# MadNLP/MadNLP.jl

Measured on AMD Instinct MI355X. Metric: IP iterations/sec + ms per factorize!/solve!, condensed KKT n≈1e4, higher is better.
Workload: dtype f64; 1 GPU; BASELINE config C3: case1354pegase-shaped sparse-condensed KKT, one instance; N=11192, m=16646, nnz(K)=68688; step = compress_J+compress_H+build_kkt+factorize (n_f=1) + inertia fetch + 2 solve_linear_system per instance; algorithm=BUNCHKAUFMAN (device: static-pivot LDL^T), outer_block=0, batch_per_gpu=1, batch_api=n/a (one instance), parallelism=1 GPU(s) x 1 independent instance(s)

## Files before the change

include/madnlp_hip.h:

```cpp
#ifndef MADNLP_HIP_H
#define MADNLP_HIP_H

#include <stdint.h>

#ifdef __cplusplus
extern "C" {
#endif

#define MNK_VERSION 100

enum { MNK_HOST = 0, MNK_DEVICE = 1 };

enum { MNK_BUNCHKAUFMAN = 1, MNK_LU = 2, MNK_QR = 3, MNK_CHOLESKY = 4, MNK_LDL = 5, MNK_EVD = 6 };

typedef struct mnk_ctx mnk_ctx;
typedef struct mnk_sc mnk_sc;
typedef struct mnk_dc mnk_dc;
typedef struct mnk_ls mnk_ls;

int mnk_version(void);
const char* mnk_last_error_string(void);
int mnk_ctx_create(int device, void* stream, mnk_ctx** out);
int mnk_ctx_destroy(mnk_ctx* ctx);
int mnk_ctx_synchronize(mnk_ctx* ctx);
// ... 193 lines not shown
int mnk_ipm_vec_copy(mnk_ipm* ipm, double* dst, const double* src, int64_t n);
int mnk_ipm_vec_fill(mnk_ipm* ipm, double* v, int64_t n, double value);
int mnk_ipm_vec_axpby(mnk_ipm* ipm, double* out, double a, const double* x, double b, const double* y, int64_t n);
int mnk_ipm_vec_scatter_axpy(mnk_ipm* ipm, double* y, const int64_t* idx, double a, const double* x, int64_t n);
int mnk_ipm_vec_gather(mnk_ipm* ipm, double* out, double a, const double* x, const int64_t* idx, int64_t n);
int mnk_ipm_bound_dual_axpy(mnk_ipm* ipm, double* zl, double* zu, double a, const double* dzl, const double* dzu);
int mnk_ipm_bound_dual_fill(mnk_ipm* ipm, double* zl, double* zu, double v);
int mnk_ipm_gemv(mnk_ipm* ipm, int trans, int64_t m, int64_t n, double alpha, const double* A, int64_t lda, const double* x,
                 double beta, double* y);

int mnk_ipm_vec_mul(mnk_ipm* ipm, double* out, const double* a, const double* b, int64_t n);
int mnk_ipm_scale_cons(mnk_ipm* ipm, double* c, const double* con_scale, const double* slack, const int64_t* slack_pos,
                       int64_t ns, const double* rhs, int64_t m);
int mnk_ipm_scale_grad(mnk_ipm* ipm, double* f, int64_t n, int64_t ntot, double factor);

typedef struct mnk_opf mnk_opf;
int mnk_opf_create(mnk_ctx* ctx, int64_t nbus, int64_t ngen, int64_t nbranch, const int32_t* fr, const int32_t* to,
                   const int32_t* gen_bus, const double* arc_coef, const double* bus_data, const double* gen_cost,
                   mnk_opf** out);
int mnk_opf_destroy(mnk_opf* opf);
int mnk_opf_sizes(mnk_opf* opf, int64_t* n, int64_t* m, int64_t* nnzj, int64_t* nnzh);
int mnk_opf_obj_terms(mnk_opf* opf, const double* x, double* terms );
int mnk_opf_grad(mnk_opf* opf, const double* x, double* g);
int mnk_opf_cons(mnk_opf* opf, const double* x, double* c);
int mnk_opf_jac_coord(mnk_opf* opf, const double* x, double* jac);
int mnk_opf_hess_coord(mnk_opf* opf, const double* x, const double* y, double obj_weight, double* hess);

typedef struct mnk_tape mnk_tape;
int mnk_tape_create(mnk_ctx* ctx, int64_t n, int64_t m, void* out);
int mnk_tape_destroy(void* tape);
int mnk_tape_add_pattern(void* tape, int kind , int64_t R, int k, int q,
                         const int32_t* var_index, const double* params, const int32_t* rows,
                         int64_t ninstr0, const int32_t* code0, int64_t nconst0, const double* consts0, int64_t nout0,
                         const int32_t* out_operand0, const int32_t* out_j0, const int32_t* out_l0, int nslot0,
                         int64_t ninstr1, const int32_t* code1, int64_t nconst1, const double* consts1, int64_t nout1,
                         const int32_t* out_operand1, const int32_t* out_j1, const int32_t* out_l1, int nslot1,
                         int64_t ninstr2, const int32_t* code2, int64_t nconst2, const double* consts2, int64_t nout2,
                         const int32_t* out_operand2, const int32_t* out_j2, const int32_t* out_l2, int nslot2);
int mnk_tape_finalize(void* tape);
int mnk_tape_sizes(void* tape, int64_t* n, int64_t* m, int64_t* nterms, int64_t* nnzj, int64_t* nnzh);
int mnk_tape_extended(void* tape, int* mask);
int mnk_tape_get_structure(void* tape, int32_t* jac_I, int32_t* jac_J, int32_t* hess_I, int32_t* hess_J);
int mnk_tape_obj_terms(void* tape, const double* x, double* terms );
int mnk_tape_grad(void* tape, const double* x, double* g);
int mnk_tape_cons(void* tape, const double* x, double* c);
int mnk_tape_jac_coord(void* tape, const double* x, double* jac);
int mnk_tape_hess_coord(void* tape, const double* x, const double* y, double obj_weight, double* hess);

typedef struct mnk_schur mnk_schur;
int mnk_schur_create(mnk_ctx* ctx, int64_t ns_local, int64_t blk, int64_t nd, int algo, mnk_schur** out);
int mnk_schur_destroy(mnk_schur* h);
int mnk_schur_set_block(mnk_schur* h, int64_t k, const double* A_kk, int64_t lda, const double* C_dk, int64_t ldc,
                        int loc);
int mnk_schur_build_local(mnk_schur* h, const double* S0, int64_t lds0, int loc_s0, double* S_out, int64_t lds_out);
int mnk_schur_factorize_s(mnk_schur* h, const double* S, int64_t lds, int loc, int* info);
int mnk_schur_inertia_s(mnk_schur* h, int64_t* num_pos, int64_t* num_zero, int64_t* num_neg);
int mnk_schur_scenario_inertia(mnk_schur* h, int64_t k, int64_t* num_pos, int64_t* num_zero, int64_t* num_neg);
int mnk_schur_scenario_bk_info(mnk_schur* h, int64_t k, int* active, int* count);
int mnk_schur_forward(mnk_schur* h, double* rhs_k, double* contrib_d);
int mnk_schur_solve_s(mnk_schur* h, double* rhs_d);
int mnk_schur_backward(mnk_schur* h, double* rhs_k, const double* x_d);
void* mnk_schur_s_buffer(mnk_schur* h);
int mnk_schur_set_structure(mnk_schur* h, int64_t n, int64_t m, int64_t nv, int64_t nc, int64_t nnzh, const int32_t* hess_I,
                            const int32_t* hess_J, int64_t nnzj, const int32_t* jac_I, const int32_t* jac_J, int64_t n_ineq,
                            const int64_t* ind_ineq, int64_t n_eq, const int64_t* ind_eq, int index_base, int64_t ns_global,
                            const int64_t* local_scen, int own_design);
int mnk_schur_assemble(mnk_schur* h, const double* hess, const double* jac, const double* pr_diag, const double* du_diag, int loc);
void* mnk_schur_s0_buffer(mnk_schur* h);
int mnk_schur_get_block(mnk_schur* h, int64_t k, double* A_kk, double* C_dk, double* S0);
int mnk_schur_solve(mnk_schur* h, double* rhs_k, double* rhs_d, int loc);

int mnk_ls_debug_solve_trace(mnk_ls* ls, unsigned long long* out, int64_t n);

int mnk_ls_debug_dag_state(mnk_ls* ls, int* flags, int64_t nflags, int* chain, int64_t nchain, int* have);

int mnk_debug_grid_at_launch(int cu_first, int num_cu, int first, int per_cu);
int mnk_debug_shader_clock(mnk_ctx* ctx, double* mhz);

int mnk_debug_dag_tasks(int ntile, int chunk, int band_tiles, int js2, int taper0, int* out, int cap, int* first_phase);
int mnk_debug_dag_merged_tasks(int ntile, int chunk, int band_tiles, int js2, int taper0, int fill, int ninst, int period,
                               int* out, int cap);
int mnk_debug_dag_deal(int ntile, int chunk, int band_tiles, int js2, int taper0, int fill, int ninst, int period, int nq, int gang,
                       int* tasks_out, int* order, int cap, int* off, int* first_phase);

int mnk_sc_debug_tile_env(mnk_sc* sc, int64_t order, int32_t* out, int cap);
int mnk_debug_tile_env_csc(int64_t n, const int32_t* colptr, const int32_t* rowval, int index_base, int32_t* out, int cap);
int mnk_sc_debug_tile_envh(mnk_sc* sc, int64_t order, int32_t* out, int cap);
int mnk_debug_tile_envh_csc(int64_t n, const int32_t* colptr, const int32_t* rowval, int index_base, int32_t* out, int cap);
int mnk_debug_envh_ksteps(int ntile, int chunk, int band_tiles, int js2, int taper0, const int* env, const int* envh, int64_t* count);

#ifdef __cplusplus
}
#endif
#endif
```

madnlp.jl_amd/_lib.py:

```python
from __future__ import annotations

import ctypes as C
import os
import subprocess

_HERE = os.path.dirname(os.path.abspath(__file__))
CSRC = os.path.join(_HERE, "csrc")
LIBDIR = os.path.join(_HERE, "lib")
LIBPATH = os.path.join(LIBDIR, "libmadnlp_hip.so")
_LIB_OVERRIDE = os.environ.get("MNK_LIBPATH")
SOURCES = ["gemm_f64.hip", "dag.hip", "factor.hip", "solve.hip", "ls.hip", "sparse_kkt.hip", "dense_kkt.hip", "bk.hip", "schur.hip", "ipm_vec.hip", "opf_eval.hip", "qr.hip", "lu.hip", "evd.hip", "qn.hip", "tape_eval.hip", "nlp_scale.hip"]
HEADERS = ["common.h", "ls.h", "kkt_vec.h", "gemm_tile.h", "leaf64.h", "ipm_handle.h", os.path.join("..", "..", "include", "madnlp_hip.h")]

MNK_HOST, MNK_DEVICE = 0, 1
MNK_BUNCHKAUFMAN, MNK_LU, MNK_QR, MNK_CHOLESKY, MNK_LDL, MNK_EVD = 1, 2, 3, 4, 5, 6
MNK_SC_JT, MNK_SC_HESS, MNK_SC_AUG, MNK_SC_DIAGBUF = 0, 1, 2, 3
MNK_QN_BFGS, MNK_QN_DAMPED_BFGS = 1, 2


def _stale() -> bool:
    if not os.path.exists(LIBPATH):
        return True
    t = os.path.getmtime(LIBPATH)
    deps = [os.path.join(CSRC, s) for s in SOURCES + HEADERS]
# ... 128 lines not shown
    "mnk_ipm_populate_RR_nn": (C.c_int, [_vp, _vp, _vp, C.c_int64, C.c_double, C.c_double]),
    "mnk_ipm_initialize_robust_restorer": (C.c_int, [_vp, _vp, _vp, C.c_int64, C.c_double, C.c_double, _vp, _vp, _vp, _vp, _vp, _vp, _vp, _vp]),
    "mnk_ipm_set_f_RR": (C.c_int, [_vp, _vp, _vp, _vp, _vp, C.c_double]),
    "mnk_ipm_set_aug_rhs_RR": (C.c_int, [_vp, _vp, _vp, _vp, _vp, _vp, _vp, _vp, _vp, _vp, _vp, C.c_int64, _vp, _vp, _vp, C.c_double, C.c_double, _vp, _vp, _vp, _vp]),
    "mnk_ipm_finish_aug_solve_RR": (C.c_int, [_vp, _vp, _vp, _vp, _vp, _vp, _vp, _vp, _vp, _vp, _vp, C.c_int64, C.c_double, C.c_double]),
    "mnk_ipm_reset_bound_dual_1": (C.c_int, [_vp, _vp, _vp, C.c_int64, C.c_double, C.c_double]),
    "mnk_ipm_set_initial_bounds": (C.c_int, [_vp, _vp, _vp, C.c_int64, C.c_double]),
    "mnk_ipm_set_initial_rhs": (C.c_int, [_vp, _vp, _vp, _vp, _vp, _vp, C.c_int64, _vp, _vp]),
    "mnk_ipm_set_aug_rhs_ifr": (C.c_int, [_vp, _vp, C.c_int64, _vp, _vp, _vp, _vp]),
    "mnk_ipm_set_g_ifr": (C.c_int, [_vp, _vp, _vp, _vp, _vp, _vp, _vp, C.c_double]),
    "mnk_ipm_initialize_variables": (C.c_int, [_vp, _vp, _vp, _vp, C.c_int64, C.c_double, C.c_double]),
    "mnk_ipm_get_dot": (C.c_int, [_vp, _vp, _vp, C.c_int64, C.POINTER(C.c_double)]),
    "mnk_ipm_get_sum": (C.c_int, [_vp, _vp, C.c_int64, C.POINTER(C.c_double)]),
    "mnk_ipm_get_norm2": (C.c_int, [_vp, _vp, C.c_int64, C.POINTER(C.c_double)]),
    "mnk_ipm_vec_copy": (C.c_int, [_vp, _vp, _vp, C.c_int64]),
    "mnk_ipm_vec_fill": (C.c_int, [_vp, _vp, C.c_int64, C.c_double]),
    "mnk_ipm_vec_axpby": (C.c_int, [_vp, _vp, C.c_double, _vp, C.c_double, _vp, C.c_int64]),
    "mnk_ipm_vec_scatter_axpy": (C.c_int, [_vp, _vp, _vp, C.c_double, _vp, C.c_int64]),
    "mnk_ipm_vec_gather": (C.c_int, [_vp, _vp, C.c_double, _vp, _vp, C.c_int64]),
    "mnk_ipm_bound_dual_axpy": (C.c_int, [_vp, _vp, _vp, C.c_double, _vp, _vp]),
    "mnk_ipm_bound_dual_fill": (C.c_int, [_vp, _vp, _vp, C.c_double]),
    "mnk_ipm_gemv": (C.c_int, [_vp, C.c_int, C.c_int64, C.c_int64, C.c_double, _vp, C.c_int64, _vp, C.c_double, _vp]),
    "mnk_ipm_vec_mul": (C.c_int, [_vp, _vp, _vp, _vp, C.c_int64]),
    "mnk_ipm_scale_cons": (C.c_int, [_vp, _vp, _vp, _vp, _vp, C.c_int64, _vp, C.c_int64]),
    "mnk_ipm_scale_grad": (C.c_int, [_vp, _vp, C.c_int64, C.c_int64, C.c_double]),
    "mnk_opf_create": (C.c_int, [_vp, C.c_int64, C.c_int64, C.c_int64, _vp, _vp, _vp, _vp, _vp, _vp, C.POINTER(_vp)]),
    "mnk_opf_destroy": (C.c_int, [_vp]),
    "mnk_opf_sizes": (C.c_int, [_vp, _i64p, _i64p, _i64p, _i64p]),
    "mnk_opf_obj_terms": (C.c_int, [_vp, _vp, _vp]),
    "mnk_opf_grad": (C.c_int, [_vp, _vp, _vp]),
    "mnk_opf_cons": (C.c_int, [_vp, _vp, _vp]),
    "mnk_opf_jac_coord": (C.c_int, [_vp, _vp, _vp]),
    "mnk_opf_hess_coord": (C.c_int, [_vp, _vp, _vp, C.c_double, _vp]),
    "mnk_tape_create": (C.c_int, [_vp, C.c_int64, C.c_int64, _vp]),
    "mnk_tape_destroy": (C.c_int, [_vp]),
    "mnk_tape_add_pattern": (C.c_int, [_vp, C.c_int, C.c_int64, C.c_int, C.c_int, _vp, _vp, _vp]
                             + [C.c_int64, _vp, C.c_int64, _vp, C.c_int64, _vp, _vp, _vp, C.c_int] * 3),
    "mnk_tape_finalize": (C.c_int, [_vp]),
    "mnk_tape_sizes": (C.c_int, [_vp, _i64p, _i64p, _i64p, _i64p, _i64p]),
    "mnk_tape_extended": (C.c_int, [_vp, _vp]),
    "mnk_tape_get_structure": (C.c_int, [_vp, _vp, _vp, _vp, _vp]),
    "mnk_tape_obj_terms": (C.c_int, [_vp, _vp, _vp]),
    "mnk_tape_grad": (C.c_int, [_vp, _vp, _vp]),
    "mnk_tape_cons": (C.c_int, [_vp, _vp, _vp]),
    "mnk_tape_jac_coord": (C.c_int, [_vp, _vp, _vp]),
    "mnk_tape_hess_coord": (C.c_int, [_vp, _vp, _vp, C.c_double, _vp]),
    "mnk_sc_set_aug_RR": (C.c_int, [_vp, _vp, _vp, _vp, _vp, _vp, _vp, _vp, _vp, _vp, _vp, C.c_double, C.c_double, C.c_double]),
    "mnk_dc_set_aug_RR": (C.c_int, [_vp, _vp, _vp, _vp, _vp, _vp, _vp, _vp, _vp, _vp, _vp, C.c_double, C.c_double, C.c_double]),
    "mnk_ls_bk_info": (C.c_int, [_vp, C.POINTER(C.c_int), C.POINTER(C.c_int), _vp, _vp]),
    "mnk_ls_get_stat": (C.c_int, [_vp, C.c_char_p, C.POINTER(C.c_double)]),
    "mnk_sc_set_bounds": (C.c_int, [_vp, C.c_int64, _vp, C.c_int64, _vp, C.c_int]),
    "mnk_sc_set_barrier_terms": (C.c_int, [_vp, _vp, _vp, _vp, _vp, _vp, C.c_int]),
    "mnk_sc_solve_kkt": (C.c_int, [_vp, _vp, _vp, C.c_int]),
    "mnk_sc_mul": (C.c_int, [_vp, _vp, _vp, C.c_double, C.c_double, C.c_int]),
    "mnk_dc_set_bounds": (C.c_int, [_vp, C.c_int64, _vp, C.c_int64, _vp, C.c_int]),
    "mnk_dc_set_barrier_terms": (C.c_int, [_vp, _vp, _vp, _vp, _vp, _vp, C.c_int]),
    "mnk_dc_solve_kkt": (C.c_int, [_vp, _vp, _vp, C.c_int]),
    "mnk_dc_mul": (C.c_int, [_vp, _vp, _vp, C.c_double, C.c_double, C.c_int]),
    "mnk_schur_create": (C.c_int, [_vp, C.c_int64, C.c_int64, C.c_int64, C.c_int, C.POINTER(_vp)]),
    "mnk_schur_destroy": (C.c_int, [_vp]),
    "mnk_schur_set_block": (C.c_int, [_vp, C.c_int64, _vp, C.c_int64, _vp, C.c_int64, C.c_int]),
    "mnk_schur_build_local": (C.c_int, [_vp, _vp, C.c_int64, C.c_int, _vp, C.c_int64]),
    "mnk_schur_factorize_s": (C.c_int, [_vp, _vp, C.c_int64, C.c_int, C.POINTER(C.c_int)]),
    "mnk_schur_inertia_s": (C.c_int, [_vp, _i64p, _i64p, _i64p]),
    "mnk_schur_scenario_inertia": (C.c_int, [_vp, C.c_int64, _i64p, _i64p, _i64p]),
    "mnk_schur_scenario_bk_info": (C.c_int, [_vp, C.c_int64, C.POINTER(C.c_int), C.POINTER(C.c_int)]),
    "mnk_schur_forward": (C.c_int, [_vp, _vp, _vp]),
    "mnk_schur_solve_s": (C.c_int, [_vp, _vp]),
    "mnk_schur_backward": (C.c_int, [_vp, _vp, _vp]),
    "mnk_schur_s_buffer": (C.c_void_p, [_vp]),
    "mnk_schur_set_structure": (C.c_int, [_vp, C.c_int64, C.c_int64, C.c_int64, C.c_int64, C.c_int64, _vp, _vp, C.c_int64, _vp, _vp,
                                          C.c_int64, _vp, C.c_int64, _vp, C.c_int, C.c_int64, _vp, C.c_int]),
    "mnk_schur_assemble": (C.c_int, [_vp, _vp, _vp, _vp, _vp, C.c_int]),
    "mnk_schur_s0_buffer": (_vp, [_vp]),
    "mnk_schur_get_block": (C.c_int, [_vp, C.c_int64, _vp, _vp, _vp]),
    "mnk_schur_solve": (C.c_int, [_vp, _vp, _vp, C.c_int]),
    "mnk_ls_debug_solve_trace": (C.c_int, [_vp, _vp, C.c_int64]),
    "mnk_ls_debug_dag_state": (C.c_int, [_vp, _vp, C.c_int64, _vp, C.c_int64, _vp]),
    "mnk_debug_grid_at_launch": (C.c_int, [C.c_int, C.c_int, C.c_int, C.c_int]),
    "mnk_debug_shader_clock": (C.c_int, [_vp, _vp]),
    "mnk_debug_dag_tasks": (C.c_int, [C.c_int, C.c_int, C.c_int, C.c_int, C.c_int, _vp, C.c_int, _vp]),
    "mnk_debug_dag_merged_tasks": (C.c_int, [C.c_int] * 8 + [_vp, C.c_int]),
    "mnk_debug_dag_deal": (C.c_int, [C.c_int] * 10 + [_vp, _vp, C.c_int, _vp, _vp]),
    "mnk_sc_debug_tile_env": (C.c_int, [_vp, C.c_int64, _vp, C.c_int]),
    "mnk_debug_tile_env_csc": (C.c_int, [C.c_int64, _vp, _vp, C.c_int, _vp, C.c_int]),
    "mnk_sc_debug_tile_envh": (C.c_int, [_vp, C.c_int64, _vp, C.c_int]),
    "mnk_debug_tile_envh_csc": (C.c_int, [C.c_int64, _vp, _vp, C.c_int, _vp, C.c_int]),
    "mnk_debug_envh_ksteps": (C.c_int, [C.c_int] * 5 + [_vp, _vp, _vp]),
    "mnk_factorize_batch_begin": (C.c_int, []),
    "mnk_factorize_batch_end": (C.c_int, []),
    "mnk_solve_batch_begin": (C.c_int, []),
    "mnk_solve_batch_end": (C.c_int, []),
    "mnk_release_idle_streams": (C.c_int, [C.c_int]),
    "mnk_sc_step_batch": (C.c_int, [C.c_int, _vp, _vp, _vp, _vp, _vp, _vp, C.c_int]),
    "mnk_ls_inertia_batch": (C.c_int, [C.c_int, _vp, _i64p, _i64p, _i64p]),
    "mnk_ls_solve_batch": (C.c_int, [C.c_int, _vp, _vp, C.c_int]),
    "mnk_gemm_nt": (C.c_int, [_vp, C.c_int, C.c_int64, C.c_int64, C.c_int64, _vp, C.c_int64, _vp,
                              C.c_int64, _vp, C.c_int64]),
}


def lib():
    global _lib
    if _lib is not None:
        return _lib
    if not os.path.exists(LIBPATH):
        raise ImportError(
            f"{LIBPATH} is missing: run `python -c 'import __graft_entry__ as g; g.build()'` "
            "(hipcc --offload-arch=gfx950).  There is no CPU fallback for the KKT hot path.")
    try:
        import torch
    except Exception:
        pass
    l = C.CDLL(_LIB_OVERRIDE if _LIB_OVERRIDE and os.path.exists(_LIB_OVERRIDE) else LIBPATH)
    for name, (res, args) in SIGNATURES.items():
        f = getattr(l, name)
        f.restype = res
        f.argtypes = args
    _lib = l
    return l


class HipError(RuntimeError):
    pass


def check(rc: int, what: str = ""):
    if rc != 0:
        msg = lib().mnk_last_error_string()
        raise HipError(f"{what} failed (rc={rc}): {msg.decode() if msg else ''}")
```

madnlp.jl_amd/csrc/common.h:

```cpp
#pragma once
#include <hip/hip_runtime.h>
#include <cstdint>
#include <cstdlib>
#include <cstdio>
#include <cstring>
#include <mutex>
#include <string>
#include <vector>

#include "../../include/madnlp_hip.h"

namespace mnk {

void set_error(const char* fmt, ...);

#define MNK_HIP(call)                                                                   \
    do {                                                                                \
        hipError_t e_ = (call);                                                         \
        if (e_ != hipSuccess) {                                                         \
            mnk::set_error("%s:%d: %s -> %s", __FILE__, __LINE__, #call, hipGetErrorString(e_)); \
            return -2;                                                                  \
        }                                                                               \
    } while (0)

// ... 91 lines not shown
    void release() {
        if (p) {
            LaunchLock lock;
            quiesce_persistent();
            (void)hipFree(p);
        }
        p = nullptr;
        n = 0;
    }
    ~DevBuf() { release(); }
};

}

struct mnk_ctx {
    int device = 0;
    hipStream_t stream = nullptr;
    bool own_stream = false;
    hipStream_t sp = nullptr, su = nullptr;
    int panel_cus = 0;
    hipStream_t sp_dag = nullptr, su_dag = nullptr;
    hipStream_t sp_dagB = nullptr, su_dagB = nullptr;
    bool shared_dag_streams = false;
    int dag_cus = 0;
    hipStream_t sp_dag2 = nullptr, su_dag2 = nullptr;
    int dag_cus2 = 0;
    hipEvent_t ev_a = nullptr, ev_b = nullptr;
    hipStream_t s_fill = nullptr;
    std::vector<hipEvent_t> ev_panel, ev_next, ev_next2, ev_bdone;
    int num_cu = 256;
    int cu_first = 0;
    int total_cu = 256;
    bool partitioned = false;
    void* persist_slot = nullptr;
    int children = 0;
    bool released = false;
};
int mnk_masked_stream_pair(mnk_ctx* ctx, int chain_cus, hipStream_t* sp, hipStream_t* su);
int mnk_ctx_ensure_panel_streams(mnk_ctx* ctx);
int mnk_ctx_ensure_dag(mnk_ctx* ctx);
int mnk_ctx_ensure_dag2(mnk_ctx* ctx);
int mnk_ctx_ensure_batch_streams(mnk_ctx* ctx);
int mnk_solve_warmup(hipStream_t s);
int mnk_ctx_bulk_wgs(const mnk_ctx* ctx, int first, int per_cu);
int mnk_dag_warmup(hipStream_t* streams, int n, int nwg);
int mnk_live_contexts(int device);
int mnk_persist_begin(mnk_ctx* ctx, hipStream_t s);
int mnk_persist_end(mnk_ctx* ctx, hipStream_t s, int rc);
void mnk_ctx_child_added(mnk_ctx* ctx);
void mnk_ctx_child_gone(mnk_ctx* ctx);

namespace mnk {
struct PpDag {
    int* front;
    const int* af;
    int ntile;
    int need_front;
    int front_from;
    int af_tilecol;
    long spin_limit;
    unsigned long long* trace;
    unsigned long long* vmax;
    int* dbg;
};
}

namespace mnk {

int launch_gemm_nt(hipStream_t s, int mode, int64_t M, int64_t N, int64_t K,
                   const double* A, int64_t lda, const double* B, int64_t ldb,
                   double* C, int64_t ldc, const double* colscale, double* C2, int64_t ldc2,
                   const int* info_flag);
struct TrsmBatchRec { double* X; double* V; const double* dblk; const double* inv16; const double* dinv; const int* info; };
struct GemmBatchRec { const double* A; const double* B; double* C; const int* info; };
int launch_gemm_nt_batch(hipStream_t s, int64_t M, int64_t N, int64_t K, const GemmBatchRec* recs_dev, int nbatch, int64_t lda,
                         int64_t ldb, int64_t ldc);
int launch_gemm_nt_lower_small(hipStream_t s, int64_t M, int64_t N, int64_t K, const double* A, int64_t lda,
                               const double* B, int64_t ldb, double* C, int64_t ldc, const int* info_flag);
int gemm_nt_lower_tiles(int64_t M, int64_t N);
int launch_gemm_nt_queue(hipStream_t s, int64_t M, int64_t N, int64_t K, const double* A, int64_t lda,
                         const double* B, int64_t ldb, double* C, int64_t ldc, int* counter, int cus,
                         const int* info_flag);

int dag_build_tasks(int ntile, int chunk, int band_tiles, int js2, std::vector<int>& out, int taper0, std::vector<int>* ready);
int dag_add_fill_tasks(int ntile, std::vector<int>& tasks, std::vector<int>& ready, int n1);
void dag_merge_tasks(const std::vector<int>& tasks, const std::vector<int>& ready, int ninst, int period, std::vector<int>& out);
constexpr int DAG_NQ = 8;
constexpr int DAG_QHEAD_STRIDE = 32;
constexpr int DAG_QHEAD_WORDS = (DAG_NQ + 1) * DAG_QHEAD_STRIDE;
void dag_deal_tasks(const std::vector<int>& tasks, const std::vector<int>& ready, int t0, int t1, int nq, int gang, std::vector<int>& order,
                    std::vector<int>& off);
void dag_envh_count(const std::vector<int>& tasks, const int* env, const int* envh, int nenv, int64_t* count);

}
```

madnlp.jl_amd/csrc/dag.hip:

```cpp
#include <algorithm>
#include <atomic>
#include <cfloat>
#include <climits>
#include <vector>

#include "gemm_tile.h"
#include "ls.h"

namespace mnk {


struct DagInst {
    double* F;
    int64_t ld;
    double* V;
    const double* dinv;
    const double* dblk;
    const double* inv16;
    int* front;
    int* af;
    int* tprog;
    int* info;
    unsigned long long* vmax;
    double* zfill;
// ... 356 lines not shown
            if (tr) { tr[4] = wall_clock64(); s_stat[1] += tr[4] - tr[3]; }
            dag_finalize_tile<LDL>(in, row0, col0, 2 * J, smem_raw, tid, X, tr);
            if (tr) s_stat[3] += wall_clock64() - tr[4];
        } else if (!(I == J && kend > k0)) {
            v4f64 acc[4][4];
#pragma unroll
            for (int i = 0; i < 4; ++i)
#pragma unroll
                for (int j = 0; j < 4; ++j) acc[i][j] = v4f64{0.0, 0.0, 0.0, 0.0};
            if (flags & DAG_FINAL) __builtin_amdgcn_s_setprio(3);
            if (!gemm_nt_mainloop<2, 2, 4, 8>(acc, Ak, in->ld, Bk, in->ld, (kend - k0) * 16, smem_raw, tid, gate)) return false;
            if (tr) tr[1] = wall_clock64();
            if (!wait_chunk_order()) return false;
            if (kend > k0)
                gemm_nt_epilogue<2, 2, 4, 2, false, true>(acc, row0, col0, (int64_t)1 << 40, (int64_t)1 << 40, in->F, in->ld, nullptr, nullptr, 0, tid);
            if (tr) tr[3] = wall_clock64();
        } else {
            v4f64 acc[4][4];
#pragma unroll
            for (int i = 0; i < 4; ++i)
#pragma unroll
                for (int j = 0; j < 4; ++j) acc[i][j] = v4f64{0.0, 0.0, 0.0, 0.0};
            __builtin_amdgcn_s_setprio(3);
            if (!wait_chunk_order()) return false;
            gemm_nt_load_neg_lower<2, 2, 4>(acc, row0, col0, in->F, in->ld, tid);
            if (!gemm_nt_mainloop<2, 2, 4, 8>(acc, Ak, in->ld, Bk, in->ld, (kend - k0) * 16, smem_raw, tid, gate)) return false;
            if (tr) tr[1] = wall_clock64();
            gemm_nt_store_neg_lower<2, 2, 4>(acc, row0, col0, in->F, in->ld, tid);
            if (tr) tr[3] = wall_clock64();
        }
        return true;
        };
        const bool done = run_task();
        asm volatile("s_waitcnt vmcnt(0)" ::: "memory");
        __syncthreads();
        if (done && tid == 0) {
            __builtin_amdgcn_fence(__ATOMIC_RELEASE, "agent");
            asm volatile("s_waitcnt vmcnt(0)" ::: "memory");
            if (!(flags & DAG_FINAL)) {
                __hip_atomic_store(in->tprog + (int64_t)I * a.ntile + J, q + 1, __ATOMIC_RELAXED, __HIP_MEMORY_SCOPE_AGENT);
            } else if (!(flags & DAG_BANDACC)) {
                __hip_atomic_store(in->front + 2 * I, J + 1, __ATOMIC_RELAXED, __HIP_MEMORY_SCOPE_AGENT);
                __hip_atomic_store(in->front + 2 * I + 1, J + 1, __ATOMIC_RELAXED, __HIP_MEMORY_SCOPE_AGENT);
            } else {
                __hip_atomic_store(in->af + (int64_t)I * a.ntile + J, 1, __ATOMIC_RELAXED, __HIP_MEMORY_SCOPE_AGENT);
            }
            if (tr) tr[5] = wall_clock64();
        }
        __builtin_amdgcn_s_setprio(0);
        __syncthreads();
        };
        do_task((DagInstP)(uintptr_t)(a.insts + inst));
    }
}

struct DagArgs1 {
    double* F;
    int64_t ld;
    double* V;
    const double* dinv;
    const double* dblk;
    const double* inv16;
    const int4* tasks;
    int ntasks;
    int* front;
    int* af;
    int* tprog;
    int ntile;
    int* qctr;
    int* info;
    long spin_limit;
    unsigned long long* trace;
    unsigned long long* wgstat;
    unsigned long long* vmax;
    int fake_share;
    double* zfill;
    int64_t N;
    const int* env;
    const int* envgate;
    const int* envh;
    const int* qoff;
    int* qheads;
    int nq;
};

__device__ __forceinline__ int dag_pop(const int* __restrict__ qoff, int* __restrict__ qheads, int nq, int* sq) {
    const int h = sq[0];
    if (h >= 0) {
        const int beg = qoff[h], n = qoff[h + 1] - beg;
        const int i = atomicAdd(qheads + h * DAG_QHEAD_STRIDE, 1);
        if (i < n) return beg + i;
        sq[0] = -1 - h;
    }
    for (;;) {
        int best = -1, most = 0;
        for (int x = 0; x < nq; ++x) {
            const int left = qoff[x + 1] - qoff[x] - __hip_atomic_load(qheads + x * DAG_QHEAD_STRIDE, __ATOMIC_RELAXED, __HIP_MEMORY_SCOPE_AGENT);
            if (left > most) { most = left; best = x; }
        }
        if (best < 0) return INT_MAX;
        const int i = atomicAdd(qheads + best * DAG_QHEAD_STRIDE, 1);
        if (i < qoff[best + 1] - qoff[best]) {
            sq[1] += 1;
            atomicAdd(qheads + nq * DAG_QHEAD_STRIDE, 1);
            return qoff[best] + i;
        }
    }
}

template <bool LDL>
__global__ __launch_bounds__(256, 3) void dag_bulk_kernel1(DagArgs1 a) {
    extern __shared__ __attribute__((aligned(16))) char smem_raw[];
    __shared__ int s_val;
    __shared__ int s_q[2];
    if (threadIdx.x == 0) {
        unsigned xcc;
        asm volatile("s_getreg_b32 %0, hwreg(HW_REG_XCC_ID)" : "=s"(xcc));
        s_q[0] = a.nq > 0 ? (int)(xcc & 15u) % a.nq : 0;
        s_q[1] = 0;
    }
    __shared__ unsigned long long s_stat[4];
    if (threadIdx.x < 4) s_stat[threadIdx.x] = 0;
    const int* __restrict__ env = a.env != nullptr && __builtin_amdgcn_readfirstlane(*a.envgate) == 0 ? a.env : nullptr;
    const int* __restrict__ envh = env != nullptr ? a.envh : nullptr;
    __syncthreads();
    for (;;) {
        int tid = threadIdx.x;
        asm volatile("" : "+v"(tid));
        if (tid == 0)
            s_val = __hip_atomic_load(a.info, __ATOMIC_RELAXED, __HIP_MEMORY_SCOPE_AGENT) != 0
                        ? INT_MAX
                        : (a.nq > 0 ? dag_pop(a.qoff, a.qheads, a.nq, s_q) : atomicAdd(a.qctr, 1));
        __syncthreads();
        const int t = s_val;
        __syncthreads();
        if (t >= a.ntasks) {
            if (a.wgstat != nullptr && tid == 0) {
                unsigned long long* w = a.wgstat + (int64_t)blockIdx.x * 8;
                w[0] = s_stat[0]; w[1] = wall_clock64(); w[2] = s_stat[1]; w[3] = s_stat[2]; w[4] = s_stat[3];
                w[5] = a.nq > 0 ? (unsigned long long)(1 + (s_q[0] >= 0 ? s_q[0] : -1 - s_q[0])) : 0; w[6] = (unsigned long long)s_q[1];
            }
            return;
        }
        if (a.wgstat != nullptr && tid == 0) { if (s_stat[0] == 0) s_stat[0] = wall_clock64(); ++s_stat[2]; }
        const int4 tk = a.tasks[t];
        const int flags = __builtin_amdgcn_readfirstlane(tk.x) & 255, q = __builtin_amdgcn_readfirstlane(tk.x) >> 8;
        const int I = __builtin_amdgcn_readfirstlane(tk.y), J = __builtin_amdgcn_readfirstlane(tk.z) & 0xfff;
        const int kbeg = __builtin_amdgcn_readfirstlane(tk.w) & 0xffff, kend = __builtin_amdgcn_readfirstlane(tk.w) >> 16;
        const int64_t row0 = (int64_t)128 * I, col0 = (int64_t)128 * J;
        unsigned long long* tr = a.trace != nullptr && tid == 0
                                     ? a.trace + (int64_t)(a.nq > 0 ? (int)((unsigned)__builtin_amdgcn_readfirstlane(tk.z) >> 12) : t) * 8
                                     : nullptr;
        if (tr) { tr[0] = wall_clock64(); tr[6] = 0; tr[7] = 0; }
        if (flags & DAG_FILL) {
            if (a.zfill != nullptr) dag_fill_tile(&a, I, J, tid);
            continue;
        }

        int eI = 0, k0 = kbeg;
        if (env != nullptr) {
            eI = __builtin_amdgcn_readfirstlane(env[I]);
            k0 = min(kend, max(kbeg, max(eI, __builtin_amdgcn_readfirstlane(env[J]))));
        }
        int kf = 0, ks = 0;
        if (envh != nullptr && (!(flags & DAG_FINAL) || (flags & DAG_BANDACC))) {
            const int w = __builtin_amdgcn_readfirstlane(tid >> 6);
            const int hI0 = __builtin_amdgcn_readfirstlane(envh[2 * I]), hI1 = __builtin_amdgcn_readfirstlane(envh[2 * I + 1]);
            const int hJ0 = __builtin_amdgcn_readfirstlane(envh[2 * J]), hJ1 = __builtin_amdgcn_readfirstlane(envh[2 * J + 1]);
            ks = min(max(8 * max(min(hI0, hI1), min(hJ0, hJ1)) - 16 * k0, 0), 16 * (kend - k0));
            kf = (I == J && w == 2) ? INT_MAX : 8 * max((w & 1) ? hI1 : hI0, (w >> 1) ? hJ1 : hJ0) - 16 * k0 - ks;
        }
        const int nk = 16 * (kend - k0) - ks;
        int limit = 0;
        auto gate_at = [&](int kc) -> int {
            const unsigned long long w0 = tr ? wall_clock64() : 0;
            const int r = dag_wait_front(&a, a.spin_limit, 2 * I, 2 * I + 1, 2 * J, 2 * J + 1, kc, kend, &s_val);
            if (tr) { const unsigned long long w1 = wall_clock64(); tr[2] = w1; tr[6] += 1; tr[7] += w1 - w0; s_stat[1] += w1 - w0; }
            return r;
        };
        auto gate = [&](int kt) -> bool {
            if (kt < limit) return true;
            const int r = gate_at(k0 + ((kt + ks) >> 4));
            if (r < 0) return false;
            limit = (__builtin_amdgcn_readfirstlane(r) - k0) * 16 - ks;
            return true;
        };
        const double* Ak = a.F + (a.fake_share > 0 ? (int64_t)128 * (kend + I % a.fake_share) : row0) + (int64_t)(128 * k0 + 8 * ks) * a.ld;
        const double* Bk = (LDL ? a.V : a.F) + (a.fake_share > 0 ? (int64_t)128 * (kend + J % a.fake_share) : col0) + (int64_t)(128 * k0 + 8 * ks) * a.ld;
        auto wait_chunk_order = [&]() -> bool {
            if (flags & DAG_FIRST) return true;
            const int* word = a.tprog + (int64_t)I * a.ntile + J;
            const unsigned long long w0 = tr ? wall_clock64() : 0;
            if (!dag_wait_words(&a, a.spin_limit, word, q, word, q, &s_val)) return false;
            if (tr) s_stat[1] += wall_clock64() - w0;
            return true;
        };
        if ((flags & DAG_FINAL) && !(flags & DAG_BANDACC)) {
            __builtin_amdgcn_s_setprio(3);
            if (!wait_chunk_order()) return;
            if (J < eI) {
                if (kend > kbeg && gate_at(kbeg) < 0) return;
                if (LDL) dag_zero_tile(a.V, a.ld, row0, col0, tid);
                goto publish;
            }
            v4f64 X[8][2];
            {
                const int lane = tid & 63, w = tid >> 6;
                const double* Cs = a.F + (row0 + 32 * w + (lane & 15)) + (col0 + (lane >> 4)) * a.ld;
#pragma unroll
                for (int cb = 0; cb < 8; ++cb)
#pragma unroll
                    for (int r = 0; r < 4; ++r) {
                        const double* cp = Cs + (int64_t)(16 * cb + 4 * r) * a.ld;
                        X[cb][0][r] = cp[0];
                        X[cb][1][r] = cp[16];
                    }
            }
            if (kend > kbeg && gate_at(kbeg) < 0) return;
            if (kend > k0) (void)gemm_nt_mainloop3<2, 8, true>(X, Ak, a.ld, Bk, a.ld, (kend - k0) * 16, smem_raw, tid);
#pragma unroll
            for (int i = 0; i < 8; ++i) { asm volatile("" : "+v"(X[i][0])); asm volatile("" : "+v"(X[i][1])); }
            if (tr) tr[1] = tr[3] = wall_clock64();
            if (dag_wait_front(&a, a.spin_limit, 2 * J, 2 * J + 1, 2 * J, 2 * J + 1, J, J + 1, &s_val) < 0) return;
            if (tr) { tr[4] = wall_clock64(); s_stat[1] += tr[4] - tr[3]; }
            dag_finalize_tile<LDL>(&a, row0, col0, 2 * J, smem_raw, tid, X, tr);
            if (tr) s_stat[3] += wall_clock64() - tr[4];
        } else if (!(I == J && kend > k0)) {
            v4f64 acc[4][4];
#pragma unroll
            for (int i = 0; i < 4; ++i)
#pragma unroll
                for (int j = 0; j < 4; ++j) acc[i][j] = v4f64{0.0, 0.0, 0.0, 0.0};
            if (flags & DAG_FINAL) __builtin_amdgcn_s_setprio(3);
            if (!gemm_nt_mainloop<2, 2, 4, 8>(acc, Ak, a.ld, Bk, a.ld, nk, smem_raw, tid, gate, kf)) return;
            if (tr) tr[1] = wall_clock64();
            if (!wait_chunk_order()) return;
            if (kend > k0 && kf < nk)
                gemm_nt_epilogue<2, 2, 4, 2, false, true>(acc, row0, col0, (int64_t)1 << 40, (int64_t)1 << 40, a.F, a.ld, nullptr, nullptr, 0, tid);
            if (tr) tr[3] = wall_clock64();
        } else {
            v4f64 acc[4][4];
#pragma unroll
            for (int i = 0; i < 4; ++i)
#pragma unroll
                for (int j = 0; j < 4; ++j) acc[i][j] = v4f64{0.0, 0.0, 0.0, 0.0};
            __builtin_amdgcn_s_setprio(3);
            if (!wait_chunk_order()) return;
            gemm_nt_load_neg_lower<2, 2, 4>(acc, row0, col0, a.F, a.ld, tid);
            if (!gemm_nt_mainloop<2, 2, 4, 8>(acc, Ak, a.ld, Bk, a.ld, nk, smem_raw, tid, gate, kf)) return;
            if (tr) tr[1] = wall_clock64();
            gemm_nt_store_neg_lower<2, 2, 4>(acc, row0, col0, a.F, a.ld, tid);
            if (tr) tr[3] = wall_clock64();
        }
    publish:
        asm volatile("s_waitcnt vmcnt(0)" ::: "memory");
        __syncthreads();
        if (tid == 0) {
            __builtin_amdgcn_fence(__ATOMIC_RELEASE, "agent");
            asm volatile("s_waitcnt vmcnt(0)" ::: "memory");
            if (!(flags & DAG_FINAL)) {
                __hip_atomic_store(a.tprog + (int64_t)I * a.ntile + J, q + 1, __ATOMIC_RELAXED, __HIP_MEMORY_SCOPE_AGENT);
            } else if (!(flags & DAG_BANDACC)) {
                __hip_atomic_store(a.front + 2 * I, J + 1, __ATOMIC_RELAXED, __HIP_MEMORY_SCOPE_AGENT);
                __hip_atomic_store(a.front + 2 * I + 1, J + 1, __ATOMIC_RELAXED, __HIP_MEMORY_SCOPE_AGENT);
            } else {
                __hip_atomic_store(a.af + (int64_t)I * a.ntile + J, 1, __ATOMIC_RELAXED, __HIP_MEMORY_SCOPE_AGENT);
            }
            if (tr) tr[5] = wall_clock64();
        }
        __builtin_amdgcn_s_setprio(0);
        __syncthreads();
    }
}

int dag_build_tasks(int ntile, int chunk, int band_tiles, int js2, std::vector<int>& out, int taper0, std::vector<int>* ready) {
    struct T { int ready, cls, J, I, flags, q, kbeg, kend; };
    std::vector<T> ts;
    auto add_tile = [&](int I, int J, int K, bool band) {
        const int body = band ? K : std::max(0, K - 1);
        std::vector<int> cuts{body};
        int e = body;
        for (int len = taper0; len < chunk && e > 0; len *= 2) { e = std::max(0, e - len); cuts.push_back(e); }
        const int first = 1 + (I * 5 + J * 3) % chunk;
        while (e > first) { e = std::max(first, e - chunk); cuts.push_back(e); }
        if (e > 0) cuts.push_back(0);
        int q = 0;
        for (int c = (int)cuts.size() - 1; c > 0; --c, ++q) {
            const int kb = cuts[c], ke = cuts[c - 1];
            const bool last = band && ke == K;
            ts.push_back({ke, band ? 0 : 2, J, I, (band ? DAG_BANDACC : 0) | (last ? DAG_FINAL : 0) | (q == 0 ? DAG_FIRST : 0), q, kb, ke});
        }
        if (!band) ts.push_back({K, 1, J, I, DAG_FINAL | (q == 0 ? DAG_FIRST : 0), q, body, K});
    };
    for (int Jt = 0; Jt < ntile; ++Jt) {
        const int Js = Jt / 2;
        const int bt = Js >= js2 ? ntile : band_tiles;
        for (int I = 2 * Js + bt; I < ntile; ++I) add_tile(I, Jt, Jt, false);
        if (2 * Js - 2 > 0)
            for (int I = std::max(2 * Js, Jt); I < 2 * Js + bt && I < ntile; ++I) add_tile(I, Jt, 2 * Js - 2, true);
    }
    std::stable_sort(ts.begin(), ts.end(), [](const T& x, const T& y) {
        if (x.ready != y.ready) return x.ready < y.ready;
        if (x.cls != y.cls) return x.cls < y.cls;
        if (x.J != y.J) return x.J < y.J;
        return x.I < y.I;
    });
    out.clear();
    out.reserve(ts.size() * 4);
    if (ready != nullptr) { ready->clear(); ready->reserve(ts.size()); }
    int n1 = 0;
    for (const T& t : ts) {
        if (t.ready <= 2 * js2) ++n1;
        if (ready != nullptr) ready->push_back(t.ready);
        out.push_back(t.flags | (t.q << 8));
        out.push_back(t.I);
        out.push_back(t.J);
        out.push_back(t.kbeg | (t.kend << 16));
    }
    return n1;
}

int dag_add_fill_tasks(int ntile, std::vector<int>& tasks, std::vector<int>& ready, int n1) {
    const int nt = (int)(tasks.size() / 4), nfill = ntile * (ntile + 1) / 2;
    const int span = n1 > 0 ? n1 : nt;
    if (span <= 0) return n1;
    std::vector<int> out, rdy;
    out.reserve(tasks.size() + 4 * (size_t)nfill);
    rdy.reserve(ready.size() + nfill);
    int fi = 0, fj = 0, done = 0;
    auto emit_fill = [&](int r) {
        out.push_back(DAG_FILL); out.push_back(fi); out.push_back(fj); out.push_back(0);
        rdy.push_back(r);
        if (++fi >= ntile) { ++fj; fi = fj; }
        ++done;
    };
    for (int t = 0; t < nt; ++t) {
        for (int k = 0; k < 4; ++k) out.push_back(tasks[4 * t + k]);
        rdy.push_back(ready[t]);
        if (t < span)
            while (done < (int)((int64_t)(t + 1) * nfill / span)) emit_fill(ready[t]);
    }
    tasks.swap(out);
    ready.swap(rdy);
    return n1 > 0 ? n1 + nfill : 0;
}

void dag_merge_tasks(const std::vector<int>& tasks, const std::vector<int>& ready, int ninst, int period, std::vector<int>& out) {
    const int nt = (int)ready.size();
    out.clear();
    out.reserve((size_t)ninst * nt * 4);
    std::vector<int> pos(ninst, 0);
    for (;;) {
        int best = -1;
        long bkey = 0;
        for (int i = 0; i < ninst; ++i) {
            if (pos[i] >= nt) continue;
            const long key = (long)i * period + ready[pos[i]];
            if (best < 0 || key < bkey) { best = i; bkey = key; }
        }
        if (best < 0) break;
        const int t = pos[best]++;
        out.push_back(tasks[4 * t]);
        out.push_back(tasks[4 * t + 1] | (best << 16));
        out.push_back(tasks[4 * t + 2]);
        out.push_back(tasks[4 * t + 3]);
    }
}

void dag_deal_tasks(const std::vector<int>& tasks, const std::vector<int>& ready, int t0, int t1, int nq, int gang, std::vector<int>& order,
                    std::vector<int>& off) {
    nq = std::max(nq, 1);
    std::vector<std::vector<int>> qs(nq);
    std::vector<int64_t> load(nq, 0);
// ... 2 lines not shown
    auto ksteps = [&](int t) { return (tasks[4 * (size_t)t] & DAG_FILL) ? 0 : (tasks[4 * (size_t)t + 3] >> 16) - (tasks[4 * (size_t)t + 3] & 0xffff); };
    auto same = [&](int x, int y) {
        return ready[x] == ready[y] && cls(x) == cls(y) && tasks[4 * (size_t)x + 2] == tasks[4 * (size_t)y + 2] &&
               tasks[4 * (size_t)x + 3] == tasks[4 * (size_t)y + 3] && (tasks[4 * (size_t)x + 1] >> 16) == (tasks[4 * (size_t)y + 1] >> 16);
    };
    auto deal = [&](int b, int e) {
        int q = 0;
        if (gang >= 0) {
            q = rr % nq;
            for (int i = 1; i < nq; ++i)
                if (load[(rr + i) % nq] < load[q]) q = (rr + i) % nq;
            rr = q + 1;
        }
        for (int t = b; t < e; ++t) { qs[q].push_back(t); load[q] += ksteps(t); }
    };
    for (int i = t0; i < t1;) {
        int j = i + 1;
        const int c = cls(i);
        if (gang > 1 && (c == 0 || c == 2))
            while (j < t1 && same(i, j)) ++j;
        for (int b = i; b < j; b += std::max(gang, 1)) deal(b, std::min(j, b + std::max(gang, 1)));
        i = j;
    }
    order.clear();
    off.assign(1, 0);
    for (int q = 0; q < nq; ++q) {
        order.insert(order.end(), qs[q].begin(), qs[q].end());
        off.push_back((int)order.size());
    }
}

void dag_envh_count(const std::vector<int>& tasks, const int* env, const int* envh, int nenv, int64_t* count) {
    count[0] = count[1] = 0;
    for (size_t t = 0; t + 3 < tasks.size(); t += 4) {
        const int flags = tasks[t] & 255, I = tasks[t + 1] & 0xffff, J = tasks[t + 2] & 0xfff, kb = tasks[t + 3] & 0xffff, ke = tasks[t + 3] >> 16;
        if (flags & DAG_FILL) continue;
        const bool in = env != nullptr && I < nenv && J < nenv;
        const int k0 = in ? std::min(ke, std::max(kb, std::max(env[I], env[J]))) : kb;
        if (in && (flags & DAG_FINAL) && !(flags & DAG_BANDACC) && J < env[I]) continue;
        count[0] += 8 * (int64_t)(ke - k0);
        if (!in || envh == nullptr || ((flags & DAG_FINAL) && !(flags & DAG_BANDACC))) continue;
        for (int r = 0; r < 2; ++r)
            for (int c = 0; c < 2; ++c) {
                const int h0 = (I == J && r == 0 && c == 1) ? 2 * ke : std::max(envh[2 * I + r], envh[2 * J + c]);
                count[1] += std::min(2 * ke, std::max(2 * k0, h0)) - 2 * k0;
            }
    }
}

template <bool LDL>
static int launch_bulk_t(hipStream_t s, const DagArgs& a, int nwg) {
    const size_t smem = TILE3_LDS_BYTES;
    auto kern = dag_bulk_kernel<LDL>;
    static std::atomic<uint64_t> attr_devs{0};
    int dev = 0;
    MNK_HIP(hipGetDevice(&dev));
    if (!(attr_devs.load(std::memory_order_relaxed) >> (dev & 63) & 1)) {
        MNK_HIP(hipFuncSetAttribute((const void*)kern, hipFuncAttributeMaxDynamicSharedMemorySize, (int)smem));
        attr_devs.fetch_or(1ull << (dev & 63), std::memory_order_relaxed);
    }
    hipLaunchKernelGGL(kern, dim3(nwg), dim3(256), smem, s, a);
    MNK_HIP(hipGetLastError());
    return 0;
}

template <bool LDL>
static int launch_bulk1_t(hipStream_t s, const DagArgs1& a, int nwg) {
    const size_t smem = TILE3_LDS_BYTES;
    auto kern = dag_bulk_kernel1<LDL>;
    static std::atomic<uint64_t> attr_devs{0};
    int dev = 0;
    MNK_HIP(hipGetDevice(&dev));
    if (!(attr_devs.load(std::memory_order_relaxed) >> (dev & 63) & 1)) {
        MNK_HIP(hipFuncSetAttribute((const void*)kern, hipFuncAttributeMaxDynamicSharedMemorySize, (int)smem));
        attr_devs.fetch_or(1ull << (dev & 63), std::memory_order_relaxed);
    }
    hipLaunchKernelGGL(kern, dim3(nwg), dim3(256), smem, s, a);
    MNK_HIP(hipGetLastError());
    return 0;
}

static int launch_dag_bulk(hipStream_t s, bool ldl, const DagInst& one, const DagInst* insts, const int* tasks, int ntasks, int ntile,
                           int* qctr, long spin_limit, int nwg, unsigned long long* trace, unsigned long long* wgstat,
                           const int* qoff = nullptr, int* qheads = nullptr, int nq = 0) {
    if (ntasks <= 0) return 0;
    static const int fake = getenv("MNK_DAG_FAKE_SHARE") ? atoi(getenv("MNK_DAG_FAKE_SHARE")) : 0;
    if (insts == nullptr) {
        DagArgs1 a{one.F, one.ld, one.V, one.dinv, one.dblk, one.inv16, reinterpret_cast<const int4*>(tasks), ntasks, one.front, one.af,
                   one.tprog, ntile, qctr, one.info, spin_limit, trace, wgstat, one.vmax, fake, one.zfill, one.N, one.env, one.envgate, one.envh,
                   qoff, qheads, nq};
        return ldl ? launch_bulk1_t<true>(s, a, nwg) : launch_bulk1_t<false>(s, a, nwg);
    }
    DagArgs a{insts, reinterpret_cast<const int4*>(tasks), ntasks, ntile, qctr, spin_limit, trace, wgstat, fake};
    return ldl ? launch_bulk_t<true>(s, a, nwg) : launch_bulk_t<false>(s, a, nwg);
}

}

using namespace mnk;

int mnk_dag_warmup(hipStream_t* streams, int n, int nwg) {
    static mnk::DevBuf<int> ctr;
    if (!ctr.p) {
        if (ctr.alloc(4)) return -2;
        MNK_HIP(hipMemset(ctr.p, 0, 4 * sizeof(int)));
    }
    for (int i = 0; i < n; ++i) {
        if (streams[i] == nullptr) continue;
        mnk::DagArgs1 a1{};
        a1.qctr = ctr.p;
        a1.info = ctr.p + 1;
        mnk::DagArgs a{};
        a.qctr = ctr.p;
        int rc = mnk::launch_bulk1_t<true>(streams[i], a1, nwg);
        if (!rc) rc = mnk::launch_bulk1_t<false>(streams[i], a1, nwg);
        if (!rc) rc = mnk::launch_bulk_t<true>(streams[i], a, nwg);
        if (!rc) rc = mnk::launch_bulk_t<false>(streams[i], a, nwg);
        if (rc) return rc;
    }
    for (int i = 0; i < n; ++i)
        if (streams[i] != nullptr) MNK_HIP(mnk::stream_wait(streams[i]));
    return 0;
}

long mnk_ls_dag_spin_limit(const mnk_ls* ls) {
    if (ls->dag_spin_limit > 0) return ls->dag_spin_limit;
    const double n = (double)ls->Np;
    const double t_est = n * n * n / 3.0 / 50e12;
    const double polls = 10.0 * t_est / 0.17e-6;
    const double floor_polls = mnk_live_contexts(ls->ctx->device) > 1 ? 5880000.0 : 588000.0;
    return (long)std::min(16777216.0, std::max(floor_polls, polls));
}

static int bulk_xcds(const mnk_ctx* c, int first) {
    bool has[8] = {false, false, false, false, false, false, false, false};
    for (int b = std::max(first, 0); b < c->num_cu; ++b) has[(c->cu_first + b) % 8] = true;
    int n = 0;
    for (bool x : has) n += x ? 1 : 0;
    return n;
}

static mnk::DagInst dag_instance(mnk_ls* ls) {
    const int ntile = (int)(ls->Np / 128), nblk = (int)(ls->Np / NBI);
    int* front = ls->dag_flags.p + 2;
    int* af = front + nblk;
    int* tprog = af + (size_t)ntile * ntile;
    double* zfill = (ls->dag_fill && ls->dag_has_fill && ls->spare_pending && ls->fact_spare.p && !ls->spare_zeroed) ? ls->fact_spare.p : nullptr;
    const bool env = ls->envelope && ls->env_dev != nullptr && ls->env_word.p != nullptr;
    return mnk::DagInst{ls->fact.p, ls->ld, ls->algo == MNK_LDL ? ls->vfull.p : nullptr, ls->dinv.p, ls->dblk.p, ls->inv16.p,
                        front, af, tprog, ls->info_dev.p, mnk_ls_growth_word(ls), zfill, ls->N, env ? ls->env_dev : nullptr,
                        env ? ls->env_word.p + 1 : nullptr, env && ls->envelope_half ? ls->envh_dev : nullptr};
}

int mnk_ls_dag_prepare(mnk_ls* ls) {
    mnk_ctx* ctx = ls->ctx;
    hipStream_t s = ctx->stream;
    const int64_t Np = ls->Np, ld = ls->ld;
    const bool ldl = ls->algo == MNK_LDL;
    const int ntile = (int)(Np / 128), nblk = (int)(Np / NBI), nsc = (int)((Np + 255) / 256);
    const size_t nflags = (size_t)2 + nblk + 2 * (size_t)ntile * ntile;
    auto give_up = [&]() {
        (void)hipGetLastError();
        ls->dag_tasks.release();
        ls->dag_flags.release();
        ls->dag_qoff.release();
        ls->dag_qheads.release();
        ls->vfull.release();
        return 1;
    };
    if (!ls->dag_tasks.p) {
        const int64_t deep_rows = std::min<int64_t>((int64_t)ctx->dag_cus2 * NBI, ls->dag_deep_rows);
        ls->dag_js2 = (ctx->dag_cus2 > 0 && Np <= deep_rows) ? 0 : nsc;
        if (ls->dag_js2_override >= 0) ls->dag_js2 = std::min(nsc, ls->dag_js2_override);
        std::vector<int>& h = ls->dag_host_tasks;
        ls->dag_ntasks1 = mnk::dag_build_tasks(ntile, ls->dag_chunk, ls->dag_band / 2, ls->dag_js2, h, ls->dag_taper0, &ls->dag_host_ready);
        ls->dag_has_fill = ls->dag_fill && ls->prefill && Np <= mnk_ls::PREFILL_MAX_ROWS;
        if (ls->dag_has_fill && h.empty()) ls->dag_has_fill = false;
        if (ls->dag_has_fill) ls->dag_ntasks1 = mnk::dag_add_fill_tasks(ntile, h, ls->dag_host_ready, ls->dag_ntasks1);
        ls->dag_ntasks = (int)(h.size() / 4);
        std::vector<int> dev_list = h, qoff(32, 0);
        ls->dag_nq[0] = ls->dag_nq[1] = 0;
        if (ls->dag_xcd_queues && ls->dag_ntasks < (1 << 20) && ntile < 4096) {
            const int part[3] = {0, ls->dag_ntasks1, ls->dag_ntasks};
            const int chain_cus[2] = {ctx->dag_cus, ctx->dag_cus2};
            for (int ph = 0; ph < 2; ++ph) {
                const int t0 = part[ph], t1 = part[ph + 1];
                if (t1 - t0 < mnk_ctx_bulk_wgs(ctx, chain_cus[ph], 3) || bulk_xcds(ctx, chain_cus[ph]) != mnk::DAG_NQ) continue;
                std::vector<int> order, off;
                mnk::dag_deal_tasks(h, ls->dag_host_ready, t0, t1, mnk::DAG_NQ, ls->dag_gang, order, off);
                for (int p = 0; p < t1 - t0; ++p) {
                    for (int k = 0; k < 4; ++k) dev_list[4 * (size_t)(t0 + p) + k] = h[4 * (size_t)order[p] + k];
                    dev_list[4 * (size_t)(t0 + p) + 2] |= (order[p] - t0) << 12;
                }
                for (int x = 0; x <= mnk::DAG_NQ; ++x) qoff[16 * ph + x] = off[x];
                ls->dag_nq[ph] = mnk::DAG_NQ;
            }
        }
        if (ls->dag_tasks.alloc(h.size() + 4)) return give_up();
        if (!ls->dag_qoff.p && ls->dag_qoff.alloc(qoff.size())) return give_up();
        if (!ls->dag_qheads.p && ls->dag_qheads.alloc(2 * (size_t)mnk::DAG_QHEAD_WORDS)) return give_up();
        {
            mnk::H2DGuard h2d;
            if (!h.empty() && hipMemcpyAsync(ls->dag_tasks.p, dev_list.data(), dev_list.size() * sizeof(int), hipMemcpyHostToDevice, s) != hipSuccess) return give_up();
            if (hipMemcpyAsync(ls->dag_qoff.p, qoff.data(), qoff.size() * sizeof(int), hipMemcpyHostToDevice, s) != hipSuccess) return give_up();
            if (mnk::stream_wait(s) != hipSuccess) return give_up();
        }
        if (ls->dag_flags.alloc(nflags)) return give_up();
    }
    if (ldl && !ls->vfull.p && ls->vfull.alloc((size_t)ld * Np + SLACK)) {
        (void)hipGetLastError();
        bool ok = false;
        if (ls->fact_spare.p && !ls->spare_zeroed) {
            ls->fact_spare.release();
            ls->prefill = 0;
            ls->spare_pending = false;
            ok = ls->vfull.alloc((size_t)ld * Np + SLACK) == 0;
        }
        if (!ok) return give_up();
    }
    if (ls->dag_trace_on) {
        const size_t ntr = (size_t)ls->dag_ntasks * 8 + 4096 * 8 + 1024 * 8;
        if (ls->dag_trace.n < ntr && ls->dag_trace.alloc(ntr)) return give_up();
    }
    return 0;
}

int mnk_ls_run_factorization_dag(mnk_ls* ls) {
    mnk_ctx* ctx = ls->ctx;
    hipStream_t s = ctx->stream;
    const int64_t Np = ls->Np;
    const bool ldl = ls->algo == MNK_LDL;
    const int ntile = (int)(Np / 128), nblk = (int)(Np / NBI), nsc = (int)((Np + 255) / 256);
    const size_t nflags = (size_t)2 + nblk + 2 * (size_t)ntile * ntile;
    MNK_REQUIRE(ls->dag_tasks.p && ls->dag_flags.p && (!ldl || ls->vfull.p), "task-DAG schedule: mnk_ls_dag_prepare was not called");
    const mnk::DagInst inst = dag_instance(ls);
    ls->dag_filled = inst.zfill != nullptr;
    ls->env_used = inst.env != nullptr;
    ls->envh_used = inst.envh != nullptr;
    hipLaunchKernelGGL(mnk::dag_reset_kernel, dim3((unsigned)std::min<size_t>((nflags + 1023) / 1024, 64)), dim3(256), 0, s,
                       ls->dag_flags.p, (int64_t)nflags, ls->info_dev.p, inst, (mnk::DagInst*)nullptr, (const mnk::SmallSysRec*)nullptr,
                       ls->env_word.p, ls->dag_qheads.p, ls->dag_qheads.p ? 2 * mnk::DAG_QHEAD_WORDS : 0);
    ls->env_armed = false;
    int* qctr = ls->dag_flags.p;
    int* front = inst.front;
    const long spin_limit = mnk_ls_dag_spin_limit(ls);
    unsigned long long* trace = nullptr;
    if (ls->dag_trace_on && ls->dag_trace.p) {
        const size_t ntr = (size_t)ls->dag_ntasks * 8 + 4096 * 8 + 1024 * 8;
        MNK_HIP(hipMemsetAsync(ls->dag_trace.p, 0, ntr * sizeof(unsigned long long), s));
        trace = ls->dag_trace.p;
    }
    const int js2 = ls->dag_js2;
    auto phase = [&](hipStream_t sp, hipStream_t su, int chain_cus, int task0, int ntask, int* counter, int js_begin, int js_end,
                     unsigned strips) -> int {
        const bool small = js_begin == 0 && js_end == nsc && js2 == 0;
        if (small) sp = s;
        MNK_HIP(hipEventRecord(ctx->ev_a, s));
        if (!small) MNK_HIP(hipStreamWaitEvent(sp, ctx->ev_a, 0));
        MNK_HIP(hipStreamWaitEvent(su, ctx->ev_a, 0));
        mnk::PpDag dag{front, inst.af, ntile, 0, 0, -1, spin_limit, trace ? trace + (size_t)ls->dag_ntasks * 8 + (size_t)js_begin * 8 * 16 : nullptr,
                  mnk_ls_growth_word(ls), ls->dag_debug ? ls->dag_dbg.p : nullptr};
        int rc = mnk_launch_pchain(ls, sp, dag, js_begin, js_end, strips);
        if (rc) return rc;
        const int ph = (int)(counter - qctr), nq = ls->dag_nq[ph];
        MNK_REQUIRE(nq == 0 || (ntask >= mnk_ctx_bulk_wgs(ctx, chain_cus, 3) && bulk_xcds(ctx, chain_cus) == nq),
                    "task-DAG schedule: the bulk grid does not cover the XCDs the task list was dealt for");
        rc = mnk::launch_dag_bulk(su, ldl, inst, nullptr, ls->dag_tasks.p + 4 * (size_t)task0, ntask, ntile, counter, spin_limit,
                                  std::min(ntask, mnk_ctx_bulk_wgs(ctx, chain_cus, 3)), trace ? trace + 8 * (size_t)task0 : nullptr,
                                  trace ? trace + (size_t)ls->dag_ntasks * 8 + 4096 * 8 + (task0 > 0 ? 512 * 8 : 0) : nullptr,
                                  ls->dag_qoff.p + 16 * ph, ls->dag_qheads.p + ph * mnk::DAG_QHEAD_WORDS, nq);
        if (rc) return rc;
        if (js_begin == 0 && js_end > 0) {
            const int64_t safe = std::min<int64_t>(js_end, std::max<int64_t>(0, (ntile - ls->dag_band / 2 - 1) / 2)) & ~(int64_t)1;
            if (strips == (unsigned)ls->dag_band && safe > 0) {
                rc = mnk_ls_invert_blocks(ls, su, 0, safe);
                if (rc) return rc;
                ls->inv_done = safe;
            }
        }
        if (small) {
            rc = mnk_ls_invert_blocks(ls, s, 0, nsc);
            if (rc) return rc;
            ls->inv_done = nsc;
        }
        if (!small) MNK_HIP(hipEventRecord(ctx->ev_a, sp));
        MNK_HIP(hipEventRecord(ctx->ev_b, su));
        if (!small) MNK_HIP(hipStreamWaitEvent(s, ctx->ev_a, 0));
        MNK_HIP(hipStreamWaitEvent(s, ctx->ev_b, 0));
        return 0;
    };
    if (js2 > 0) {
        int rc = phase(ctx->sp_dag, ctx->su_dag, ctx->dag_cus, 0, ls->dag_ntasks1, qctr, 0, std::min(js2, nsc),
                       (unsigned)std::min<int64_t>(ls->dag_band, Np / NBI));
        if (rc) return rc;
    }
    if (js2 < nsc) {
        const int64_t rows2 = Np - 256 * (int64_t)js2;
        MNK_REQUIRE(ctx->sp_dag2 != nullptr, "task-DAG schedule: the deep-band streams are missing");
        int rc = phase(ctx->sp_dag2, ctx->su_dag2, ctx->dag_cus2, ls->dag_ntasks1, ls->dag_ntasks - ls->dag_ntasks1,
                       qctr + 1, js2, nsc, (unsigned)(rows2 / NBI));
        if (rc) return rc;
    }
    return 0;
}

namespace {
struct BatchState {
    int depth = 0;
    bool active = false;
    std::vector<mnk_ls*> pend;
};
thread_local BatchState t_batch;

struct BatchBuffers {
    mnk::DevBuf<int> tasks;
    mnk::DevBuf<int> qctr;
    mnk::DevBuf<char> insts, pcsys, aux;
    char* stage = nullptr;
    size_t stage_bytes = 0;
    hipEvent_t stage_ev = nullptr;
    int ntile = 0, ninst = 0, period = 0, chunk = 0, taper0 = 0, band = 0, ntasks = 0;
    bool fill = false;
    hipEvent_t ev[4] = {nullptr, nullptr, nullptr, nullptr};
};
BatchBuffers g_batch[64];
}

bool mnk_batch_active() { return t_batch.active; }

bool mnk_batch_defer(mnk_ls* ls) {
    if (!t_batch.active) return false;
    const int nsc = (int)((ls->Np + 255) / 256);
    if (ls->algo_now != 5 || (ls->dag_js2 != nsc && ls->dag_js2 != 0) || ls->dag_trace_on || ls->ctx->partitioned) return false;
    if (mnk_ctx_ensure_batch_streams(ls->ctx) != 0) (void)hipGetLastError();
    if (!ls->ctx->sp_dagB) return false;
    if (!ls->ev_defer && hipEventCreateWithFlags(&ls->ev_defer, hipEventDisableTiming) != hipSuccess) { (void)hipGetLastError(); return false; }
    if (hipEventRecord(ls->ev_defer, ls->ctx->stream) != hipSuccess) { (void)hipGetLastError(); return false; }
    ls->deferred = true;
    t_batch.pend.push_back(ls);
    return true;
}

static void batch_mark_done(mnk_ls* ls) {
    ls->factorized = true;
    ls->info_valid = false;
    ls->bk_active = false;
    ls->deferred = false;
}

static int batch_run_group(std::vector<mnk_ls*>& g) {
    mnk_ls* l0 = g[0];
    mnk_ctx* c0 = l0->ctx;
    hipStream_t h = c0->stream;
    MNK_HIP(hipSetDevice(c0->device));
    const int64_t Np = l0->Np;
    const bool ldl = l0->algo == MNK_LDL;
    const int ntile = (int)(Np / 128), nsc = (int)((Np + 255) / 256), ninst = (int)g.size();
    const size_t nflags = (size_t)2 + (size_t)(Np / NBI) + 2 * (size_t)ntile * ntile;
    for (mnk_ls* ls : g)
        if (ls->ctx->stream != h) MNK_HIP(hipStreamWaitEvent(h, ls->ev_defer, 0));
    int rc = mnk_persist_begin(c0, h);
    if (rc) return rc;
    auto body = [&]() -> int {
        BatchBuffers& B = g_batch[c0->device & 63];
        const int period = (ntile + 1) / 2;
        if (B.ntile != ntile || B.ninst != ninst || B.period != period || B.chunk != l0->dag_chunk || B.taper0 != l0->dag_taper0 ||
            B.band != l0->dag_band || B.fill != l0->dag_has_fill || !B.tasks.p) {
            std::vector<int> merged;
            mnk::dag_merge_tasks(l0->dag_host_tasks, l0->dag_host_ready, ninst, period, merged);
            if (B.tasks.alloc(merged.size() + 4)) return -2;
            { mnk::H2DGuard h2d; MNK_HIP(hipMemcpy(B.tasks.p, merged.data(), merged.size() * sizeof(int), hipMemcpyHostToDevice)); }
            if (!B.qctr.p && B.qctr.alloc(4)) return -2;
            if (B.insts.alloc(sizeof(mnk::DagInst) * (size_t)ninst)) return -2;
            for (hipEvent_t& e : B.ev)
                if (!e) MNK_HIP(hipEventCreateWithFlags(&e, hipEventDisableTiming));
            B.ntile = ntile; B.ninst = ninst; B.period = period; B.chunk = l0->dag_chunk; B.taper0 = l0->dag_taper0;
            B.band = l0->dag_band; B.fill = l0->dag_has_fill; B.ntasks = (int)(merged.size() / 4);
        }
        std::vector<mnk::DagInst> hin;
        mnk::DagInst* insts_dev = reinterpret_cast<mnk::DagInst*>(B.insts.p);
        for (mnk_ls* ls : g) {
            hin.push_back(dag_instance(ls));
            ls->dag_filled = hin.back().zfill != nullptr;
// ... 252 lines not shown
bool mnk_ls_pending_elsewhere(const mnk_ls* ls) {
    return ls->deferred && std::find(t_batch.pend.begin(), t_batch.pend.end(), ls) == t_batch.pend.end();
}

int mnk_ls_sync_deferred_fact(mnk_ls* ls) {
    if (!ls->deferred) return 0;
    if (std::find(t_batch.pend.begin(), t_batch.pend.end(), ls) == t_batch.pend.end()) {
        set_error("a factorize! call of this solver is pending in a batch that another thread opened (mnk_factorize_batch_end must come first)");
        return -1;
    }
    return batch_flush();
}

extern "C" int mnk_factorize_batch_begin(void) {
    ++t_batch.depth;
    t_batch.active = true;
    return 0;
}

extern "C" int mnk_factorize_batch_end(void) {
    if (t_batch.depth <= 0) { set_error("mnk_factorize_batch_end: no batch is open on this thread"); return -1; }
    if (--t_batch.depth > 0) return 0;
    t_batch.active = false;
    return batch_flush();
}

extern "C" int mnk_debug_dag_tasks(int ntile, int chunk, int band_tiles, int js2, int taper0, int* out, int cap, int* first_phase) {
    if (ntile <= 0 || chunk <= 0 || band_tiles <= 0 || taper0 <= 0) return -1;
    std::vector<int> h;
    const int n1 = mnk::dag_build_tasks(ntile, chunk, band_tiles, js2, h, taper0, nullptr);
    const int n = (int)(h.size() / 4);
    if (first_phase != nullptr) *first_phase = n1;
    if (out != nullptr)
        for (int i = 0; i < std::min(n, cap) * 4; ++i) out[i] = h[i];
    return n;
}

extern "C" int mnk_debug_dag_merged_tasks(int ntile, int chunk, int band_tiles, int js2, int taper0, int fill, int ninst, int period,
                                          int* out, int cap) {
    if (ntile <= 0 || chunk <= 0 || band_tiles <= 0 || taper0 <= 0 || ninst <= 0 || period < 0) return -1;
    std::vector<int> h, ready, merged;
    int n1 = mnk::dag_build_tasks(ntile, chunk, band_tiles, js2, h, taper0, &ready);
    if (fill) n1 = mnk::dag_add_fill_tasks(ntile, h, ready, n1);
    mnk::dag_merge_tasks(h, ready, ninst, period, merged);
    const int n = (int)(merged.size() / 4);
    if (out != nullptr)
        for (int i = 0; i < std::min(n, cap) * 4; ++i) out[i] = merged[i];
    return n;
}

extern "C" int mnk_debug_dag_deal(int ntile, int chunk, int band_tiles, int js2, int taper0, int fill, int ninst, int period, int nq,
                                  int gang, int* tasks_out, int* order, int cap, int* off, int* first_phase) {
    if (ntile <= 0 || chunk <= 0 || band_tiles <= 0 || taper0 <= 0 || ninst <= 0 || period < 0 || nq <= 0 || nq > 64 || gang == 0) return -1;
    std::vector<int> h, ready;
    int n1 = mnk::dag_build_tasks(ntile, chunk, band_tiles, js2, h, taper0, &ready);
    if (fill) n1 = mnk::dag_add_fill_tasks(ntile, h, ready, n1);
    if (ninst > 1) {
        std::vector<int> merged, mready, pos(ninst, 0);
        mnk::dag_merge_tasks(h, ready, ninst, period, merged);
        for (size_t t = 0; t < merged.size() / 4; ++t) { const int i = merged[4 * t + 1] >> 16; mready.push_back(i * period + ready[pos[i]++]); }
        h.swap(merged);
        ready.swap(mready);
        n1 = (int)ready.size();
    }
    const int n = (int)ready.size();
    if (first_phase != nullptr) *first_phase = n1;
    const int part[3] = {0, n1, n};
    int written = 0;
    for (int ph = 0; ph < 2; ++ph) {
        std::vector<int> ord, o;
        mnk::dag_deal_tasks(h, ready, part[ph], part[ph + 1], nq, gang, ord, o);
        for (int x = 0; x <= nq; ++x)
            if (off != nullptr) off[ph * (nq + 1) + x] = part[ph] + o[x];
        for (int v : ord) {
            if (order != nullptr && written < cap) order[written] = v;
            ++written;
        }
    }
    if (tasks_out != nullptr)
        for (int i = 0; i < std::min(n, cap) * 4; ++i) tasks_out[i] = h[i];
    return n;
}

extern "C" int mnk_debug_envh_ksteps(int ntile, int chunk, int band_tiles, int js2, int taper0, const int* env, const int* envh, int64_t* count) {
    if (ntile <= 0 || chunk <= 0 || band_tiles <= 0 || taper0 <= 0 || count == nullptr) return -1;
    std::vector<int> h;
    (void)mnk::dag_build_tasks(ntile, chunk, band_tiles, js2, h, taper0, nullptr);
    mnk::dag_envh_count(h, env, envh, ntile, count);
    return (int)(h.size() / 4);
}
```

madnlp.jl_amd/csrc/factor.hip:

```cpp
#include <atomic>
#include <type_traits>
#include <atomic>
#include <cfloat>
#include <chrono>
#include <cmath>
#include <cstdlib>

#include "ls.h"
#include "leaf64.h"

namespace mnk {

template <bool LDL, int NS>
__device__ __forceinline__ void trsm64_mfma_body(double* __restrict__ F, int64_t ld, int64_t j0, int64_t Np,
                                                 const double* __restrict__ Dblk, const double* __restrict__ inv16,
                                                 const double* __restrict__ dinv, double* __restrict__ W, int64_t ldw,
                                                 int64_t wcol, const int* __restrict__ info,
                                                 unsigned long long* __restrict__ vmax) {
    if (*info != 0) return;
    const int lane = threadIdx.x & 63, wave = threadIdx.x >> 6;
    const int l15 = lane & 15, l4 = lane >> 4;
    const int64_t r0 = j0 + 64 + ((int64_t)blockIdx.x * 4 + wave) * (16 * NS);
    if (r0 >= Np) return;
    double Ln[6][4];
// ... 616 lines not shown
    }
}

__global__ void pc_set_sys_kernel(PcSys rec, PcSys* __restrict__ dst) { *dst = rec; }

template <bool LDL>
__global__ __launch_bounds__(256) void linv64_kernel(double* __restrict__ F, int64_t ld,
                                                      const double* __restrict__ Dblk,
                                                      double* __restrict__ Linv, const int* __restrict__ info, int blk0,
                                                      const SmallSysRec* __restrict__ recs = nullptr) {
    __shared__ double Lt[64 * 64];
    __shared__ double rd[64];
    __shared__ double xk[2][64];
    if (recs != nullptr) {
        const SmallSysRec r = recs[blockIdx.z];
        F = r.F; ld = r.ld; Dblk = r.dblk; Linv = r.linv; info = r.info;
    }
    if (*info != 0) return;
    const int64_t blk = (int64_t)blockIdx.x + blk0;
    const int64_t j0 = blk * 64;
    const int c = threadIdx.x & 63;
    const int p = __builtin_amdgcn_readfirstlane(threadIdx.x >> 6);
    const double* A = Dblk + blk * 4096;
    double* Fd = F + j0 + j0 * ld;
#pragma unroll 4
    for (int i = 0; i < 16; ++i) {
        const int q = 4 * i + p, lane = c;
        const double v = lane >= q ? A[lane + 64 * q] : 0.0;
        if (lane >= q) Fd[lane + (int64_t)q * ld] = v;
        Lt[q * 64 + lane] = lane > q ? v : (lane == q ? (LDL ? 1.0 : v) : 0.0);
        if (lane == q) rd[q] = LDL ? 1.0 : 1.0 / v;
    }
    __syncthreads();
    double s[16];
#pragma unroll
    for (int i = 0; i < 16; ++i) s[i] = (4 * i + p == c) ? 1.0 : 0.0;
#pragma unroll
    for (int k = 0; k < 64; ++k) {
        if ((k & 3) == p) {
            const double x = s[k >> 2] * rd[k];
            s[k >> 2] = x;
            xk[k & 1][c] = x;
        }
        __syncthreads();
        const double x = xk[k & 1][c];
#pragma unroll
        for (int i = 0; i < 16; ++i)
            if (4 * i + 3 > k) {
                const int r = 4 * i + p;
                if (r > k) s[i] -= Lt[k * 64 + r] * x;
            }
    }
    __syncthreads();
#pragma unroll
    for (int i = 0; i < 16; ++i) Lt[c * 64 + 4 * i + p] = s[i];
    __syncthreads();
    double* out = Linv + blk * 4096;
#pragma unroll 4
    for (int i = 0; i < 16; ++i) out[c + 64 * (4 * i + p)] = Lt[c + 64 * (4 * i + p)];
}

__global__ void publish_info_kernel(const unsigned long long* __restrict__ inertia, const int* __restrict__ info,
                                    unsigned long long* __restrict__ host_words) {
    if (threadIdx.x == 0 && blockIdx.x == 0) {
        for (int i = 0; i < 3; ++i) __hip_atomic_store(host_words + i, inertia[i], __ATOMIC_RELAXED, __HIP_MEMORY_SCOPE_SYSTEM);
        for (int i = 0; i < 3; ++i) __hip_atomic_store(host_words + 4 + i, 0ull, __ATOMIC_RELAXED, __HIP_MEMORY_SCOPE_SYSTEM);
        __hip_atomic_store(host_words + 3, (unsigned long long)(long long)*info, __ATOMIC_RELEASE, __HIP_MEMORY_SCOPE_SYSTEM);
    }
}

__global__ __launch_bounds__(1024) void finish_info_kernel(const double* __restrict__ dvec, int64_t N, const int* __restrict__ info,
                                                            unsigned long long* __restrict__ host_words,
                                                            const unsigned long long* __restrict__ amax,
                                                            const SmallSysRec* __restrict__ recs = nullptr) {
    __shared__ unsigned long long red[16][4];
    __shared__ double redm[16];
    if (recs != nullptr) {
        const SmallSysRec r = recs[blockIdx.x];
        dvec = r.dvec; N = r.ninertia; info = r.info; host_words = r.pin_dev; amax = r.amax;
    }
    unsigned long long pos = 0, zer = 0, neg = 0, chg = 0;
    double amx = 0.0;
    if (N > 0 && *info == -9) N = info[1] + 1 < N ? info[1] + 1 : N;
    for (int64_t k = threadIdx.x; k < N; k += blockDim.x) {
        const double d = dvec[k];
        if (d > 0.0) ++pos;
        else if (d < 0.0) ++neg;
        else ++zer;
        const double a = fabs(d) <= DBL_MAX ? fabs(d) : __longlong_as_double(0x7ff0000000000000LL);
        amx = fmax(amx, a);
        if (k + 1 < N && ((d > 0.0) != (dvec[k + 1] > 0.0))) ++chg;
    }
    for (int off = 32; off > 0; off >>= 1) {
        pos += __shfl_xor((long long)pos, off);
        zer += __shfl_xor((long long)zer, off);
        neg += __shfl_xor((long long)neg, off);
        chg += __shfl_xor((long long)chg, off);
        amx = fmax(amx, __shfl_xor(amx, off));
    }
    const int w = threadIdx.x >> 6;
    if ((threadIdx.x & 63) == 0) { red[w][0] = pos; red[w][1] = zer; red[w][2] = neg; red[w][3] = chg; redm[w] = amx; }
    __syncthreads();
    unsigned long long am = 0ull;
    if (amax != nullptr && threadIdx.x < 64) {
        for (int i = threadIdx.x; i < AMAX_SLOTS; i += 64) am = std::max(am, amax[AMAX_SLOT0 + AMAX_STRIDE * i]);
        for (int off = 32; off > 0; off >>= 1) am = std::max(am, (unsigned long long)__shfl_xor((long long)am, off));
        am = std::max(am, amax[0]);
    }
    if (threadIdx.x == 0) {
        const int nw = (int)(blockDim.x >> 6);
        unsigned long long t[4] = {0, 0, 0, 0};
        double m = 0.0;
        for (int i = 0; i < nw; ++i) {
            for (int j = 0; j < 4; ++j) t[j] += red[i][j];
            m = fmax(m, redm[i]);
        }
        for (int i = 0; i < 3; ++i) __hip_atomic_store(host_words + i, t[i], __ATOMIC_RELAXED, __HIP_MEMORY_SCOPE_SYSTEM);
        unsigned long long gw = 0ull;
        if (amax != nullptr) gw = std::max(amax[1], (unsigned long long)__double_as_longlong(m));
        __hip_atomic_store(host_words + 4, am, __ATOMIC_RELAXED, __HIP_MEMORY_SCOPE_SYSTEM);
        __hip_atomic_store(host_words + 5, gw, __ATOMIC_RELAXED, __HIP_MEMORY_SCOPE_SYSTEM);
        __hip_atomic_store(host_words + 6, amax != nullptr ? t[3] : 0ull, __ATOMIC_RELAXED, __HIP_MEMORY_SCOPE_SYSTEM);
        __hip_atomic_store(host_words + 7, (unsigned long long)(long long)info[1], __ATOMIC_RELAXED, __HIP_MEMORY_SCOPE_SYSTEM);
        __hip_atomic_store(host_words + 3, (unsigned long long)(long long)*info, __ATOMIC_RELEASE, __HIP_MEMORY_SCOPE_SYSTEM);
    }
}

}

using namespace mnk;

unsigned long long* mnk_ls_growth_word(mnk_ls* ls) {
    return (ls->algo == MNK_LDL && ls->bk_requested && ls->bk_fallback && ls->amax_dev.p) ? ls->amax_dev.p + 1 : nullptr;
}

constexpr int SMALL_TILES_MID = 1000;

static int factor_outer_panel_pp(mnk_ls* ls, hipStream_t s, int64_t ko, int64_t kend, double* wbase,
                                 hipEvent_t rest_ready, int64_t rest_from, const double* Vfirst, int64_t ldvfirst,
                                 int64_t Kfirst) {
    const int64_t Np = ls->Np, ld = ls->ld;
    const bool ldl = ls->algo == MNK_LDL;
    double* F = ls->fact.p;
    {
        static std::atomic<uint64_t> attr_devs{0};
        int dev = 0;
        MNK_HIP(hipGetDevice(&dev));
        if (!(attr_devs.load(std::memory_order_relaxed) >> (dev & 63) & 1)) {
            MNK_HIP(hipFuncSetAttribute((const void*)ppanel_kernel<true, 4>, hipFuncAttributeMaxDynamicSharedMemorySize, PP_LDS_BYTES));
            MNK_HIP(hipFuncSetAttribute((const void*)ppanel_kernel<false, 4>, hipFuncAttributeMaxDynamicSharedMemorySize, PP_LDS_BYTES));
            attr_devs.fetch_or(1ull << (dev & 63), std::memory_order_relaxed);
        }
    }
    constexpr int NBs = 4;
    const int64_t ws = (int64_t)NBI * NBs;
    const int epoch16 = ls->epoch * 16;
    bool waited = rest_ready == nullptr;
    const double* Vp = Vfirst;
    int64_t ldv = ldvfirst;
    int Kp = (int)Kfirst;
    const bool fuse_mid = ls->pp_fuse_rows > 0 && Np - ko <= ls->pp_fuse_rows;
    for (int64_t p = ko; p < kend; p += ws) {
        const int nbk = (int)std::min<int64_t>(NBs, (kend - p) / NBI);
        if (!waited && p + NBI * nbk > ko + rest_from) {
            MNK_HIP(hipStreamWaitEvent(s, rest_ready, 0));
            waited = true;
        }
        const unsigned grid = (unsigned)((Np - p) / NBI);
    unsigned long long* vmaxw = mnk_ls_growth_word(ls);
#define MNK_PP(LD, NBT)                                                                                              \
    hipLaunchKernelGGL((ppanel_kernel<LD, NBT>), dim3(grid), dim3(256), PP_LDS_BYTES, s, F, ld, p, nbk, Np, ls->dblk.p, \
                       ls->inv16.p, ls->dvec.p, ls->dinv.p, LD ? wbase : (double*)nullptr, LD ? ls->ldw : (int64_t)0,  \
                       p - ko, ls->info_dev.p, ls->pivot_tol, ls->flag_p.p + p / NBI, epoch16, ls->debug_pp_missing, Vp,  \
                       ldv, Kp, PpDag{nullptr, nullptr, 0, 0, 4, -1, 0, nullptr, vmaxw})
// ... 125 lines not shown
    }
    const bool ldl = ls->algo == MNK_LDL;
    const int epoch16 = ls->epoch * 16;
    double* V = ldl ? ls->vfull.p : nullptr;
    if (ldl)
        hipLaunchKernelGGL(pchain_kernel<true>, dim3(strips), dim3(256), PC_LDS_BYTES, sp, ls->fact.p, ls->ld, ls->Np, ls->dblk.p,
                           ls->inv16.p, ls->dvec.p, ls->dinv.p, V, ls->info_dev.p, ls->pivot_tol, ls->flag_p.p, epoch16,
                           ls->debug_pp_missing, dag, js_begin, js_end);
    else
        hipLaunchKernelGGL(pchain_kernel<false>, dim3(strips), dim3(256), PC_LDS_BYTES, sp, ls->fact.p, ls->ld, ls->Np, ls->dblk.p,
                           ls->inv16.p, ls->dvec.p, ls->dinv.p, V, ls->info_dev.p, ls->pivot_tol, ls->flag_p.p, epoch16,
                           ls->debug_pp_missing, dag, js_begin, js_end);
    MNK_HIP(hipGetLastError());
    return 0;
}

static int run_factorization_body(mnk_ls* ls);

size_t mnk_pchain_sys_bytes() { return sizeof(mnk::PcSys); }
void mnk_pchain_fill_sys(mnk_ls* ls, void* rec_host, int* front, const int* af) {
    const bool ldl = ls->algo == MNK_LDL;
    *static_cast<mnk::PcSys*>(rec_host) = mnk::PcSys{ls->fact.p, ls->ld, ls->Np, ls->dblk.p, ls->inv16.p, ls->dvec.p, ls->dinv.p,
                                                       ldl ? ls->vfull.p : nullptr, ls->info_dev.p, ls->pivot_tol, ls->flag_p.p,
                                                       ls->epoch * 16, front, af, (int)(ls->Np / 128), mnk_ls_dag_spin_limit(ls),
                                                       mnk_ls_growth_word(ls)};
}

int mnk_launch_pchain_multi(mnk_ls* const* v, int n, hipStream_t sp, hipStream_t fill_stream, void* table, int* const* front,
                            const int* const* af) {
    {
        static std::atomic<uint64_t> attr_devs{0};
        int dev = 0;
        MNK_HIP(hipGetDevice(&dev));
        if (!(attr_devs.load(std::memory_order_relaxed) >> (dev & 63) & 1)) {
            MNK_HIP(hipFuncSetAttribute((const void*)pchain_multi_kernel<true>, hipFuncAttributeMaxDynamicSharedMemorySize, PC_LDS_BYTES));
            MNK_HIP(hipFuncSetAttribute((const void*)pchain_multi_kernel<false>, hipFuncAttributeMaxDynamicSharedMemorySize, PC_LDS_BYTES));
            attr_devs.fetch_or(1ull << (dev & 63), std::memory_order_relaxed);
        }
    }
    mnk::PcSys* dst = static_cast<mnk::PcSys*>(table);
    const bool ldl = v[0]->algo == MNK_LDL;
    const int strips = (int)(v[0]->Np / NBI);
    for (int i = 0; i < n && fill_stream != nullptr; ++i) {
        mnk_ls* ls = v[i];
        mnk::PcSys rec{ls->fact.p, ls->ld, ls->Np, ls->dblk.p, ls->inv16.p, ls->dvec.p, ls->dinv.p, ldl ? ls->vfull.p : nullptr,
                       ls->info_dev.p, ls->pivot_tol, ls->flag_p.p, ls->epoch * 16, front[i], af[i], (int)(ls->Np / 128),
                       mnk_ls_dag_spin_limit(ls), mnk_ls_growth_word(ls)};
        hipLaunchKernelGGL(pc_set_sys_kernel, dim3(1), dim3(1), 0, fill_stream, rec, dst + i);
    }
    MNK_HIP(hipGetLastError());
    if (ldl)
        hipLaunchKernelGGL(pchain_multi_kernel<true>, dim3((unsigned)(n * strips)), dim3(256), PC_LDS_BYTES, sp, dst, strips);
    else
        hipLaunchKernelGGL(pchain_multi_kernel<false>, dim3((unsigned)(n * strips)), dim3(256), PC_LDS_BYTES, sp, dst, strips);
    MNK_HIP(hipGetLastError());
    return 0;
}

int mnk_ls_run_factorization(mnk_ls* ls) {
    if (ls->algo == MNK_QR) return mnk_qr_factor(ls);
    if (ls->algo == MNK_LU) return mnk_lu_factor(ls);
    if (ls->algo == MNK_EVD) return mnk_evd_factor(ls);
    mnk_ctx* ctx = ls->ctx;
    hipStream_t s = ctx->stream;
    const int64_t Np = ls->Np;
    if (ls->panel_algo >= 4 && !ls->flag_p.p) {
        if (ls->flag_p.alloc(Np / NBI + 1)) return -2;
        MNK_HIP(hipMemsetAsync(ls->flag_p.p, 0, (Np / NBI + 1) * sizeof(int), s));
    }
    ++ls->epoch;
    ls->inv_done = 0;
    ls->factor_invalid = false;
    ls->t_fact_launch_ms = mnk_host_ms();
    {
        const int want = (ls->early_reject && ls->accept_only_pd && ls->algo == MNK_LDL && ls->src_persistent) ? 1 : 0;
        if (want != ls->reject_on_device) {
            MNK_HIP(hipMemsetAsync(ls->info_dev.p + 2, want, sizeof(int), s));
            ls->reject_on_device = want;
        }
    }
    ls->algo_now = ls->panel_algo;
    ls->env_used = false;
    ls->envh_used = false;
    const int64_t min_rows = mnk_batch_active() ? std::min<int64_t>(ls->dag_min_rows, 256) : ls->dag_min_rows;
    if (ls->algo_now == 5 && (ctx->dag_cus < ls->dag_band || !ls->lookahead || Np < min_rows || Np > ls->dag_max_rows)) ls->algo_now = 4;
    if (ls->algo_now == 5 && ctx->sp_dag == nullptr && mnk_ctx_ensure_dag(ctx) != 0) { (void)hipGetLastError(); ls->algo_now = 4; }
    if (ls->algo_now == 5 && ctx->sp_dag == nullptr) ls->algo_now = 4;
    ++ls->fact_count;
    if (ls->pp_blocked && ls->fact_count >= ls->pp_retry_at) ls->pp_blocked = false;
    if (ls->algo_now >= 4 && ls->pp_blocked) ls->algo_now = 1;
    if (ls->algo_now == 5 && mnk_ls_dag_prepare(ls) != 0) ls->algo_now = 4;
    if (ls->algo_now == 5 && ls->dag_js2 < (Np + 255) / 256) {
        if (mnk_ctx_ensure_dag2(ctx) != 0) (void)hipGetLastError();
        if (ctx->sp_dag2 == nullptr) ls->algo_now = 4;
    }
    if (ls->algo_now == 5 && mnk_batch_defer(ls)) return 0;
    return mnk_ls_run_factorization_now(ls);
}

int mnk_ls_run_factorization_now(mnk_ls* ls) {
    mnk_ctx* ctx = ls->ctx;
    hipStream_t s = ctx->stream;
    const bool persistent = ls->algo_now >= 4;
    if (persistent) {
        int rc0 = mnk_persist_begin(ctx, s);
        if (rc0) return rc0;
    }
    const int rc_run = run_factorization_body(ls);
    return persistent ? mnk_persist_end(ctx, s, rc_run) : rc_run;
}

static int run_factorization_body(mnk_ls* ls) {
    mnk_ctx* ctx = ls->ctx;
    hipStream_t s = ctx->stream;
    const int64_t Np = ls->Np, ld = ls->ld;
    const bool ldl = ls->algo == MNK_LDL;
    double* F = ls->fact.p;
    const int64_t NBO = mnk_ls_effective_nbo(ls);
    if (ls->algo_now != 5) MNK_HIP(hipMemsetAsync(ls->info_dev.p, 0, 2 * sizeof(int), s));
    constexpr int64_t TAIL_ROWS = 4096, TAIL_NBO = 256;
    std::vector<int64_t> bnd{0};
    for (int64_t pos = 0; pos < Np;) {
        const bool tail = ls->lookahead && NBO < Np && Np - pos <= TAIL_ROWS && TAIL_NBO < NBO;
        pos = std::min<int64_t>(pos + (tail ? TAIL_NBO : NBO), Np);
        bnd.push_back(pos);
    }
    const int64_t npanel = (int64_t)bnd.size() - 1;
    const bool la = ls->lookahead && npanel > 1;

    if (ls->algo_now == 5) {
        int rc = mnk_ls_run_factorization_dag(ls);
        if (rc) return rc;
    } else if (!la) {
        for (int64_t ko = 0; ko < Np; ko += NBO) {
            const int64_t kend = std::min<int64_t>(ko + NBO, Np);
            int rc = factor_outer_panel(ls, s, ko, kend, ls->wbuf[0].p);
            if (rc) return rc;
            const int64_t Mt = Np - kend;
            if (Mt > 0) {
                const double* Wsrc = ldl ? ls->wbuf[0].p + kend : F + kend + ko * ld;
                rc = launch_gemm_nt(s, 2, Mt, Mt, kend - ko, Wsrc, ldl ? ls->ldw : ld, F + kend + ko * ld, ld,
                                    F + kend + kend * ld, ld, nullptr, nullptr, 0, ls->info_dev.p);
                if (rc) return rc;
            }
        }
    } else {
        { int rc_s = mnk_ctx_ensure_panel_streams(ctx); if (rc_s) return rc_s; }
        hipStream_t sp = ctx->sp, su = ctx->su;
        if ((int64_t)ctx->ev_panel.size() < npanel + 1) {
            const size_t old = ctx->ev_panel.size();
            ctx->ev_panel.resize(npanel + 1);
            ctx->ev_next.resize(npanel + 1);
            ctx->ev_next2.resize(npanel + 1);
            ctx->ev_bdone.resize(npanel + 1);
            for (size_t e = old; e < ctx->ev_panel.size(); ++e) {
                MNK_HIP(hipEventCreateWithFlags(&ctx->ev_panel[e], hipEventDisableTiming));
                MNK_HIP(hipEventCreateWithFlags(&ctx->ev_next[e], hipEventDisableTiming));
                MNK_HIP(hipEventCreateWithFlags(&ctx->ev_next2[e], hipEventDisableTiming));
                MNK_HIP(hipEventCreateWithFlags(&ctx->ev_bdone[e], hipEventDisableTiming));
            }
        }
        const int pcus = ctx->panel_cus;
        const int ucus = pcus > 0 ? ctx->num_cu - pcus : ctx->num_cu;
        const bool share = ls->share != 0;
        if (share) {
            if (ls->tile_ctr.n < 8 * ((size_t)npanel + 1)) {
// ... 8 lines not shown
        MNK_HIP(hipStreamWaitEvent(sp, ctx->ev_a, 0));
        MNK_HIP(hipStreamWaitEvent(su, ctx->ev_a, 0));
        MNK_HIP(hipEventRecord(ctx->ev_panel[0], sp));
        for (int64_t k = 0; k + 1 < npanel; ++k) {
            const int64_t ko = bnd[k], kend = bnd[k + 1];
            const int64_t Mt = Np - kend;
            if (Mt <= 0) break;
            const int64_t nnext = bnd[k + 2] - kend;
            double* wk = ls->wbuf[k & 1].p;
            const double* Wsrc = ldl ? wk + kend : F + kend + ko * ld;
            const int64_t ldws = ldl ? ls->ldw : ld;
            const int64_t Kw = kend - ko;
            MNK_HIP(hipStreamWaitEvent(su, ctx->ev_panel[k], 0));
            auto update_a = [&](hipStream_t st, int64_t c0, int64_t c1) -> int {
                const int64_t Mp = Mt - c0, Nn = c1 - c0;
                double* Cp = F + (kend + c0) + (kend + c0) * ld;
                if (gemm_nt_lower_tiles(Mp, Nn) < ls->small_tiles)
                    return launch_gemm_nt_lower_small(st, Mp, Nn, Kw, Wsrc + c0, ldws, F + kend + c0 + ko * ld, ld, Cp,
                                                      ld, ls->info_dev.p);
                return launch_gemm_nt(st, 2, Mp, Nn, Kw, Wsrc + c0, ldws, F + kend + c0 + ko * ld, ld, Cp, ld, nullptr,
                                      nullptr, 0, ls->info_dev.p);
            };
            const bool fuse_a = ls->algo_now == 4 && ls->pp_fuse_rows > 0 && Mt <= ls->pp_fuse_rows && Kw <= 512;
            constexpr int64_t OWN_COLS = 128;
            const bool own_first = !fuse_a && nnext > NBI;
            const int64_t n1 = own_first ? std::min<int64_t>(OWN_COLS, nnext - NBI) : std::min<int64_t>(256, nnext);
            const bool split_a = nnext > n1;
            if (fuse_a) {
                if (k > 0) MNK_HIP(hipStreamWaitEvent(sp, ctx->ev_bdone[k - 1], 0));
                if (split_a) {
                    rc = update_a(su, n1, nnext);
                    if (rc) return rc;
                    MNK_HIP(hipEventRecord(ctx->ev_next2[k], su));
                }
            } else if (own_first) {
                if (k > 0) MNK_HIP(hipStreamWaitEvent(sp, ctx->ev_bdone[k - 1], 0));
                rc = update_a(sp, 0, n1);
                if (rc) return rc;
                rc = update_a(su, n1, nnext);
                if (rc) return rc;
                MNK_HIP(hipEventRecord(ctx->ev_next2[k], su));
            } else {
                rc = update_a(su, 0, nnext);
                if (rc) return rc;
                MNK_HIP(hipEventRecord(ctx->ev_next[k], su));
            }
            const int64_t Mb = Mt - nnext;
            const int64_t Nb = Mb;
            bool shared_b = false;
            if (Mb > 0 && Nb > 0) {
                const int ntiles = gemm_nt_lower_tiles(Mb, Nb);
                const double t_upd = ntiles * (68.0 * (double)Kw / 512.0) / ucus;
                const double t_pan = 55.0 * (double)nnext / 64.0 * (pcus > 0 ? 64.0 / pcus : 1.0);
                shared_b = share && pcus > 0 && (t_upd > t_pan || ls->share == 2);
                if (shared_b)
                    rc = launch_gemm_nt_queue(su, Mb, Nb, Kw, Wsrc + nnext, ldws, F + kend + nnext + ko * ld, ld,
                                              F + (kend + nnext) + (kend + nnext) * ld, ld, ls->tile_ctr.p + 8 * k,
                                              ucus, ls->info_dev.p);
                else
                    rc = launch_gemm_nt(su, 2, Mb, Nb, Kw, Wsrc + nnext, ldws, F + kend + nnext + ko * ld, ld,
                                        F + (kend + nnext) + (kend + nnext) * ld, ld, nullptr, nullptr, 0,
                                        ls->info_dev.p);
                if (rc) return rc;
            }
            MNK_HIP(hipEventRecord(ctx->ev_bdone[k], su));
            if (!own_first && !fuse_a) MNK_HIP(hipStreamWaitEvent(sp, ctx->ev_next[k], 0));
            rc = factor_outer_panel(ls, sp, kend, kend + nnext, ls->wbuf[(k + 1) & 1].p,
                                    split_a ? ctx->ev_next2[k] : nullptr, own_first ? n1 : 256,
                                    fuse_a ? (ldl ? wk : F + ko * ld) : nullptr, ldws, fuse_a ? Kw : 0);
            if (rc) return rc;
            if (shared_b) {
                rc = launch_gemm_nt_queue(sp, Mb, Nb, Kw, Wsrc + nnext, ldws, F + kend + nnext + ko * ld, ld,
                                          F + (kend + nnext) + (kend + nnext) * ld, ld, ls->tile_ctr.p + 8 * k,
                                          pcus, ls->info_dev.p);
                if (rc) return rc;
            }
            MNK_HIP(hipEventRecord(ctx->ev_panel[k + 1], sp));
        }
        MNK_HIP(hipEventRecord(ctx->ev_a, sp));
        MNK_HIP(hipEventRecord(ctx->ev_b, su));
        MNK_HIP(hipStreamWaitEvent(s, ctx->ev_a, 0));
        MNK_HIP(hipStreamWaitEvent(s, ctx->ev_b, 0));
    }
    {
        int rc = mnk_ls_invert_blocks(ls, s, ls->inv_done, (Np + 255) / 256);
        if (rc) return rc;
    }
    ls->factorized = true;
    ls->info_valid = false;
    ls->bk_active = false;
    {
        int rc = mnk_ls_launch_finish_info(ls, s);
        if (rc) return rc;
    }
    return mnk_ls_prefill_spare(ls);
}

void mnk_ls_fill_small_rec(mnk_ls* ls, mnk::SmallSysRec* rec) {
    const bool lmode = ls->algo == MNK_LDL;
    const int64_t ntile = ls->Np / 128;
    rec->flags = ls->dag_flags.p;
    rec->nflags = 2 + ls->Np / NBI + 2 * ntile * ntile;
    rec->info = ls->info_dev.p;
    rec->F = ls->fact.p; rec->ld = ls->ld; rec->dblk = ls->dblk.p; rec->linv = ls->linv.p;
    rec->linv256 = ls->linv256.p; rec->linv256t = ls->linv256t.p; rec->Np = ls->Np;
    rec->dvec = ls->dvec.p; rec->ninertia = lmode ? ls->N : 0; rec->pin_dev = ls->pin_dev;
    rec->amax = mnk_ls_growth_word(ls) != nullptr ? ls->amax_dev.p : nullptr;
}

int mnk_ls_invert_blocks_batch(hipStream_t s, bool ldl, const mnk::SmallSysRec* recs_dev, int n, int64_t Np) {
    const unsigned nb = (unsigned)(Np / NBI);
    if (ldl) hipLaunchKernelGGL(linv64_kernel<true>, dim3(nb, 1, (unsigned)n), dim3(256), 0, s, (double*)nullptr, (int64_t)0, (const double*)nullptr,
                                (double*)nullptr, (const int*)nullptr, 0, recs_dev);
    else hipLaunchKernelGGL(linv64_kernel<false>, dim3(nb, 1, (unsigned)n), dim3(256), 0, s, (double*)nullptr, (int64_t)0, (const double*)nullptr,
                            (double*)nullptr, (const int*)nullptr, 0, recs_dev);
    MNK_HIP(hipGetLastError());
    return mnk_ls_build_inverses_batch(s, recs_dev, n, Np);
}

int mnk_ls_finish_info_batch(hipStream_t s, const mnk::SmallSysRec* recs_dev, int n, int threads) {
    hipLaunchKernelGGL(finish_info_kernel, dim3((unsigned)n), dim3(threads), 0, s, (const double*)nullptr, (int64_t)0, (const int*)nullptr,
                       (unsigned long long*)nullptr, (const unsigned long long*)nullptr, recs_dev);
    MNK_HIP(hipGetLastError());
    return 0;
}

int mnk_ls_launch_finish_info(mnk_ls* ls, hipStream_t s) {
    const bool lmode = ls->algo == MNK_LDL;
    const int threads = lmode ? (ls->N >= 4096 ? 1024 : 256) : 64;
    hipLaunchKernelGGL(finish_info_kernel, dim3(1), dim3(threads), 0, s, ls->dvec.p, lmode ? ls->N : (int64_t)0, ls->info_dev.p, ls->pin_dev,
                       mnk_ls_growth_word(ls) != nullptr ? ls->amax_dev.p : (const unsigned long long*)nullptr);
    MNK_HIP(hipGetLastError());
    if (!ls->ev_info) MNK_HIP(hipEventCreateWithFlags(&ls->ev_info, hipEventDisableTiming));
    MNK_HIP(hipEventRecord(ls->ev_info, s));
    ls->ev_info_recorded = true;
    return 0;
}

int mnk_ls_right_trsm_rows(mnk_ls* ls, hipStream_t s, int64_t j0, double* Xrows, double* Vrows, int64_t ldr, int64_t nrows) {
    MNK_REQUIRE(ls->factorized && !ls->bk_active && nrows % 16 == 0 && j0 % NBI == 0 && j0 < ls->Np,
                "mnk_ls_right_trsm_rows: needs a static-pivot factor, 16-row multiples and a block-aligned column");
    double* Fp = Xrows - (j0 + NBI);
    double* Wp = Vrows ? Vrows - (j0 + NBI) : nullptr;
    const unsigned grid = (unsigned)((nrows / 16 + 3) / 4);
    const double* dblk = ls->dblk.p + (j0 / NBI) * 4096;
    const double* inv16 = ls->inv16.p + (j0 / NBI) * 1024;
    if (ls->algo == MNK_LDL)
        hipLaunchKernelGGL((trsm64_mfma_kernel<true, 1>), dim3(grid), dim3(256), 0, s, Fp, ldr, j0, j0 + NBI + nrows, dblk,
                           inv16, ls->dinv.p, Wp, ldr, (int64_t)j0, ls->info_dev.p);
    else
        hipLaunchKernelGGL((trsm64_mfma_kernel<false, 1>), dim3(grid), dim3(256), 0, s, Fp, ldr, j0, j0 + NBI + nrows, dblk,
                           inv16, ls->dinv.p, (double*)nullptr, (int64_t)0, (int64_t)0, ls->info_dev.p);
    MNK_HIP(hipGetLastError());
    return 0;
}

int mnk_launch_trsm64_batch(hipStream_t s, bool ldl, const mnk::TrsmBatchRec* recs_dev, int nbatch, int64_t j0, int64_t nrows,
                            int64_t ldr) {
    if (nbatch <= 0 || nrows <= 0) return 0;
    MNK_REQUIRE(nrows % 16 == 0 && j0 % NBI == 0, "mnk_launch_trsm64_batch: 16-row multiples and a block-aligned column");
    const dim3 grid((unsigned)((nrows / 16 + 3) / 4), (unsigned)nbatch);
    if (ldl) hipLaunchKernelGGL(trsm64_mfma_batch_kernel<true>, grid, dim3(256), 0, s, recs_dev, ldr, j0, nrows);
    else hipLaunchKernelGGL(trsm64_mfma_batch_kernel<false>, grid, dim3(256), 0, s, recs_dev, ldr, j0, nrows);
    MNK_HIP(hipGetLastError());
    return 0;
}

static int bk_fallback(mnk_ls* ls) {
    hipStream_t s = ls->ctx->stream;
    int rc = ls->retransfer();
    if (rc) return rc;
    rc = mnk_ls_run_bunchkaufman(ls);
    if (rc) return rc;
    rc = mnk_ls_invert_blocks(ls, s, 0, (ls->Np + 255) / 256);
// ... 121 lines not shown
```

madnlp.jl_amd/csrc/ls.h:

```cpp
#pragma once
#include <algorithm>
#include <functional>
#include <memory>
#include <string>
#include <vector>

#include "common.h"

struct mnk_sc {
    mnk_ctx* ctx = nullptr;
    int64_t n = 0, m = 0, nnzj = 0, nnzh = 0;
    int64_t nnz_jt = 0, nnz_hess = 0, nnz_aug = 0, len_jptr = 0;
    std::vector<int32_t> jt_colptr, jt_rowval, h_colptr, h_rowval, aug_colptr, aug_rowval;
    std::vector<int32_t> tile_env;
    mnk::DevBuf<int32_t> d_tile_env;
    std::vector<int32_t> tile_envh;
    mnk::DevBuf<int32_t> d_tile_envh;
    std::vector<int64_t> jt_map, h_map;
    std::vector<int32_t> d_dst, d_src, hp_dst, hp_src, j_dst, j_c, j_k, j_l;
    mnk::DevBuf<int32_t> jt_seg_ptr, jt_seg_src, h_seg_ptr, h_seg_src;
    mnk::DevBuf<int32_t> aug_hptr, aug_hsrc;
    mnk::DevBuf<int32_t> aug_dsrc;
    mnk::DevBuf<int32_t> aug_jptr, aug_jc, aug_jk, aug_jl;
    mnk::DevBuf<int32_t> aug_row, aug_col;
// ... 13 lines not shown
    for (int64_t I = 0; I < ntile; ++I) {
        int32_t f = (int32_t)(128 * I);
        for (int64_t i = 128 * I; i < std::min<int64_t>(n, 128 * I + 128); ++i) f = std::min(f, fnz[i]);
        env[I] = f / 128;
    }
    return env;
}

inline std::vector<int32_t> mnk_tile_envelope_half(int64_t n, const int32_t* row, const int32_t* col, int64_t nnz) {
    std::vector<int32_t> fnz(n);
    for (int64_t i = 0; i < n; ++i) fnz[i] = (int32_t)i;
    for (int64_t k = 0; k < nnz; ++k)
        if (row[k] >= 0 && row[k] < n && col[k] < fnz[row[k]]) fnz[row[k]] = col[k];
    const int64_t nhalf = 2 * ((n + 127) / 128);
    std::vector<int32_t> envh(nhalf);
    for (int64_t h = 0; h < nhalf; ++h) {
        int32_t f = (int32_t)(64 * h);
        for (int64_t i = 64 * h; i < std::min<int64_t>(n, 64 * h + 64); ++i) f = std::min(f, fnz[i]);
        envh[h] = f / 64;
    }
    return envh;
}

struct mnk_dc {
    mnk_ctx* ctx = nullptr;
    int condensed = 1;
    bool mirror_pending = false;
    int64_t n = 0, m = 0, ns = 0, n_eq = 0, order = 0;
    std::vector<int64_t> ind_ineq, ind_eq;
    mnk::DevBuf<int64_t> d_ind_ineq, d_ind_eq;
    mnk::DevBuf<double> hess, jac, aug, pr_diag, du_diag, diag_buffer;
    mnk::DevBuf<double> jis;
    int64_t ld_jis = 0, kpad = 0, npad = 0;
    void* extra = nullptr;
    void* qn = nullptr;
    std::shared_ptr<int> alive = std::make_shared<int>(0);
};
void mnk_dc_qn_release(mnk_dc* dc);

constexpr int EVD_BLOCK = 32;

struct mnk_ls {
    mnk_ctx* ctx = nullptr;
    int64_t N = 0, Np = 0, ld = 0, ldw = 0, nbo = 512;
    bool nbo_auto = true;
    int algo = MNK_LDL;
    double pivot_tol = 0.0;
    int lookahead = 1;
    int share = 1;
    int small_tiles = 400;
    int64_t single_rows = 2560;
    mnk::DevBuf<int> tile_ctr;
    mnk::DevBuf<double> fact, wbuf[2], linv, dblk, inv16, linv256, linv256t, dvec, dinv, xwork;
    mnk::DevBuf<double> fact_spare;
    hipEvent_t ev_spare = nullptr, ev_free = nullptr;
    bool spare_zeroed = false, spare_pending = false;
    int prefill = 1;
    static constexpr int64_t PREFILL_MAX_ROWS = 24576;
    int epoch = 0;
    mnk::DevBuf<int> flag_p;
    int algo_now = 1;
    bool pp_blocked = false;
    int64_t fact_count = 0, pp_retry_at = 0, pp_backoff = 16;
    int pp_fallbacks = 0;
    int last_timeout_site = 0;
    double stall_ms_total = 0.0;
    double t_fact_launch_ms = 0.0;
    int64_t pp_fuse_rows = 4096;
    mnk::DevBuf<int> dag_tasks;
    int dag_ntasks = 0, dag_ntasks1 = 0, dag_js2 = 0;
    std::vector<int> dag_host_tasks, dag_host_ready;
    int dag_fill = 1;
    bool dag_has_fill = false;
    bool dag_filled = false;
    hipEvent_t ev_info = nullptr;
    bool ev_info_recorded = false;
    hipEvent_t ev_defer = nullptr;
    bool deferred = false;
    int dag_xcd_queues = 1;
    int dag_gang = 4;
    int dag_nq[2] = {0, 0};
    mnk::DevBuf<int> dag_qoff;
    mnk::DevBuf<int> dag_qheads;
    mnk::DevBuf<int> dag_flags;
    mnk::DevBuf<double> vfull;
    mnk::DevBuf<unsigned long long> dag_trace;
    bool dag_trace_on = false;
    int64_t inv_done = 0;
    int dag_band = 16;
    int dag_taper0 = 2;
    long dag_spin_limit = 0;
    int dag_chunk = 64;
    int64_t dag_min_rows = 1280;
    int64_t dag_deep_rows = 5376;
    int envelope = 1;
    const int32_t* env_dev = nullptr;
    std::vector<int32_t> env_host;
    mnk::DevBuf<int32_t> env_own;
    int envelope_half = 1;
    const int32_t* envh_dev = nullptr;
    std::vector<int32_t> envh_host;
    mnk::DevBuf<int32_t> envh_own;
    bool envh_used = false;
    mnk::DevBuf<int> env_word;
    bool env_used = false;
    bool env_armed = false;
    int64_t dag_max_rows = 30720;
    int panel_algo = 5;
    int persistent_solve = 1;
    int solve512 = 0;
    std::vector<std::string> env_keys;
    int dag_js2_override = -1;
    int linv_mfma = 1;
    mnk::DevBuf<double> linv512, linv512t, linv512tmp;
    int pub_next = 0;
    bool pub_clean[2] = {false, false};
    int* solve_abort = nullptr;
    long ps_spin_limit = 6000000;
    int debug_pp_missing = -1;
    int debug_ps_missing = -1;
    mnk::DevBuf<unsigned long long> solve_trace;
    mnk::DevBuf<int> info_dev;
    mnk::DevBuf<unsigned long long> inertia_dev;
    unsigned long long* pin = nullptr;
    unsigned long long* pin_dev = nullptr;
    bool bk_requested = false;
    int bk_fallback = 1;
    int early_reject = 0;
    int reject_on_device = -1;
    bool src_persistent = false;
    bool factor_invalid = false;
    int64_t early_rejects = 0, early_reject_col = -1, early_reject_redone = 0;
    int probe = 1;
    mnk_ls* probe_ls = nullptr;
    int64_t probe_order = 0;
    int64_t probe_hint_col = -1;
    int probe_since_hint = 1 << 20;
    bool probe_last_rejected = false;
    int64_t probe_hits = 0, probe_misses = 0;
    int accept_only_pd = 0;
    double bk_growth_tol = 64.0, bk_growth_tol_qd = 1e8;
    double last_growth = 0.0;
    int64_t last_sign_changes = 0;
    mnk::DevBuf<unsigned long long> amax_dev;
    bool bk_active = false;
    int bk_count = 0;
    std::function<int()> retransfer;
    mnk::DevBuf<int> bk_perm, bk_ptype;
    mnk::DevBuf<double> bk_doff, bk_dcoup, bk_work;
    mnk::DevBuf<char> bk_state;
    mnk::DevBuf<double> bk_wv, bk_tmp;
    mnk::DevBuf<unsigned long long> bk_msg;
    mnk::DevBuf<int> bk_aux;
    int bk_panel_wgs = 0;
    int bk_max_wgs = 0;
    long bk_spin_limit = 1L << 21;
    int debug_bk_missing = -1;
    bool bk_multi_last = false, bk_mw_blocked = false;
    int bk_mw_fallbacks = 0;
    bool factorized = false, info_valid = false;
    int dag_debug = 0;
    mnk::DevBuf<int> dag_dbg;
    std::vector<int> dbg_flags, dbg_chain;
    bool spare_by_dag = false;
    int info = 0;
    int64_t npos = 0, nzero = 0, nneg = 0;
// ... 72 lines not shown
```

madnlp.jl_amd/csrc/ls.hip:

```cpp
#include <cstdarg>
#include <cstdlib>
#include <atomic>
#include <map>
#include <mutex>

#include <cfloat>
#include "ls.h"

namespace mnk {

static thread_local std::string g_err;
void set_error(const char* fmt, ...) {
    char buf[1024];
    va_list ap;
    va_start(ap, fmt);
    vsnprintf(buf, sizeof(buf), fmt, ap);
    va_end(ap);
    g_err = buf;
}

__global__ __launch_bounds__(256) void fill_lower_kernel(double* __restrict__ F, int64_t ld, int64_t N, int64_t Np) {
    const int64_t col = blockIdx.x;
    const int64_t first = (col / PAD) * PAD;
    const int64_t r = first + ((int64_t)blockIdx.y * 256 + threadIdx.x) * 2;
// ... 600 lines not shown
    delete ls;
    mnk_ctx_child_gone(ctx);
    return 0;
}

int mnk_ls_set_option(mnk_ls* ls, const char* key, double value) {
    MNK_REQUIRE(ls && key, "mnk_ls_set_option: NULL argument");
    { int rc_d = mnk_ls_sync_deferred(ls); if (rc_d) return rc_d; }
    for (const std::string& k : ls->env_keys)
        if (k == key) {
            static std::mutex warn_mutex;
            static std::vector<std::string> warned;
            std::lock_guard<std::mutex> lock(warn_mutex);
            if (std::find(warned.begin(), warned.end(), k) == warned.end()) {
                warned.push_back(k);
                fprintf(stderr, "madnlp_hip: set_option('%s', %g) ignored: the option is pinned by MNK_OPTIONS / MNK_PANEL_ALGO / "
                                "MNK_PERSISTENT_SOLVE for this process (query: get_stat(\"pinned:%s\"))\n", key, value, key);
            }
            return 0;
        }
    if (!strcmp(key, "pivot_tol")) { ls->pivot_tol = value; return 0; }
    if (!strcmp(key, "envelope_half")) { ls->envelope_half = value != 0.0; return 0; }
    if (!strcmp(key, "envelope")) { ls->envelope = value != 0.0; return 0; }
    if (!strcmp(key, "dag_js2")) { ls->dag_js2_override = (int)value; return 0; }
    if (!strcmp(key, "outer_block")) {
        int64_t v = (int64_t)value;
        MNK_REQUIRE(v == 0 || (v >= NBI && v % NBI == 0), "outer_block must be 0 (by size) or a positive multiple of 64");
        ls->nbo_auto = v == 0;
        if (v > 0) ls->nbo = v;
        ls->wbuf[0].release();
        ls->wbuf[1].release();
        return 0;
    }
    if (!strcmp(key, "solve512")) { ls->solve512 = value != 0; return 0; }
    if (!strcmp(key, "linv_mfma")) { ls->linv_mfma = value != 0.0; return 0; }
    if (!strcmp(key, "prefill")) { ls->prefill = value != 0; return 0; }
    if (!strcmp(key, "single_rows")) {
        ls->single_rows = (int64_t)value;
        ls->wbuf[0].release();
        ls->wbuf[1].release();
        return 0;
    }
    if (!strcmp(key, "lookahead")) { ls->lookahead = value != 0.0; return 0; }
    if (!strcmp(key, "share")) { ls->share = (int)value; return 0; }
    if (!strcmp(key, "small_tiles")) { ls->small_tiles = (int)value; return 0; }
    if (!strcmp(key, "panel_algo")) {
        MNK_REQUIRE((int)value == 1 || (int)value == 4 || (int)value == 5, "panel_algo must be 1, 4 or 5");
        ls->panel_algo = (int)value;
        return 0;
    }
    if (!strcmp(key, "pp_fuse_rows")) { ls->pp_fuse_rows = (int64_t)value; return 0; }
    if (!strcmp(key, "dag_min_rows")) { ls->dag_min_rows = (int64_t)value; return 0; }
    if (!strcmp(key, "dag_taper0")) {
        MNK_REQUIRE(value >= 1.0 && value <= 16.0, "dag_taper0 must be in 1..16");
        ls->dag_taper0 = (int)value;
        ls->dag_tasks.release();
        return 0;
    }
    if (!strcmp(key, "dag_chunk")) {
        MNK_REQUIRE(value >= 1.0 && value <= 64.0, "dag_chunk must be in 1..64");
        ls->dag_chunk = (int)value;
        ls->dag_tasks.release();
        return 0;
    }
    if (!strcmp(key, "dag_band")) {
        MNK_REQUIRE(value >= 8.0 && value <= 64.0 && (int)value % 4 == 0 && (double)(int)value == value, "dag_band must be a multiple of 4 in 8..64");
        ls->dag_band = (int)value;
        ls->dag_tasks.release();
        return 0;
    }
    if (!strcmp(key, "dag_spin_limit")) {
        MNK_REQUIRE(value >= 1024.0, "dag_spin_limit must be at least 1024");
        ls->dag_spin_limit = (long)value;
        return 0;
    }
    if (!strcmp(key, "dag_fill")) { ls->dag_fill = value != 0.0; ls->dag_tasks.release(); return 0; }
    if (!strcmp(key, "dag_xcd_queues")) { ls->dag_xcd_queues = value != 0.0; ls->dag_tasks.release(); return 0; }
    if (!strcmp(key, "dag_gang")) {
        MNK_REQUIRE(value <= 64.0 && value != 0.0 && (double)(int)value == value, "dag_gang must be an integer in 1..64 (or negative)");
        ls->dag_gang = (int)value;
        ls->dag_tasks.release();
        return 0;
    }
    if (!strcmp(key, "dag_trace")) { ls->dag_trace_on = value != 0.0; return 0; }
    if (!strcmp(key, "dag_max_rows")) { ls->dag_max_rows = (int64_t)value; return 0; }
    if (!strcmp(key, "dag_deep_rows")) { ls->dag_deep_rows = (int64_t)value; ls->dag_tasks.release(); return 0; }
    if (!strcmp(key, "bk_fallback")) { ls->bk_fallback = (int)value; return 0; }
    if (!strcmp(key, "bk_panel_wgs")) {
        MNK_REQUIRE(value == 0.0 || value == 1.0, "bk_panel_wgs must be 0 or 1");
        ls->bk_panel_wgs = (int)value;
        return 0;
    }
    if (!strcmp(key, "accept_only_pd")) { ls->accept_only_pd = value != 0; return 0; }
    if (!strcmp(key, "probe")) { ls->probe = value != 0; return 0; }
    if (!strcmp(key, "early_reject")) { ls->early_reject = value != 0; return 0; }
    if (!strcmp(key, "dag_debug")) {
        ls->dag_debug = value != 0.0;
        if (ls->dag_debug && !ls->dag_dbg.p) {
            if (ls->dag_dbg.alloc(8 * 128 + 16 * 1024)) return -2;
            MNK_HIP(hipMemset(ls->dag_dbg.p, 0, (8 * 128 + 16 * 1024) * sizeof(int)));
        }
        return 0;
    }
    if (!strcmp(key, "bk_max_wgs")) {
        MNK_REQUIRE(value >= 0.0 && value <= 256.0, "bk_max_wgs must be in 0..256");
        ls->bk_max_wgs = (int)value;
        return 0;
    }
    if (!strcmp(key, "bk_spin_limit")) {
        MNK_REQUIRE(value >= 1024.0, "bk_spin_limit must be at least 1024");
        ls->bk_spin_limit = (long)value;
        return 0;
    }
    if (!strcmp(key, "debug_bk_missing")) { ls->debug_bk_missing = (int)value; return 0; }
    if (!strcmp(key, "bk_growth_tol")) {
        MNK_REQUIRE(value > 1.0, "bk_growth_tol must be > 1");
        ls->bk_growth_tol = value;
        return 0;
    }
    if (!strcmp(key, "bk_growth_tol_qd")) {
        MNK_REQUIRE(value > 1.0, "bk_growth_tol_qd must be > 1");
        ls->bk_growth_tol_qd = value;
        return 0;
    }
    if (!strcmp(key, "persistent_solve")) { ls->persistent_solve = value != 0.0; return 0; }
    if (!strcmp(key, "ps_spin_limit")) {
        MNK_REQUIRE(value >= 1024.0, "ps_spin_limit must be at least 1024");
        ls->ps_spin_limit = (long)value;
        return 0;
    }
    if (!strcmp(key, "debug_pp_missing")) { ls->debug_pp_missing = (int)value; return 0; }
    if (!strcmp(key, "debug_ps_missing")) { ls->debug_ps_missing = (int)value; return 0; }
    if (!strcmp(key, "solve_trace")) {
        if (value != 0.0) {
            int rc = ls->solve_trace.alloc((size_t)(ls->Np / 64) * 8);
            if (rc) return rc;
            MNK_HIP(hipMemset(ls->solve_trace.p, 0, (size_t)(ls->Np / 64) * 8 * sizeof(unsigned long long)));
        } else {
            ls->solve_trace.release();
        }
        return 0;
    }
    set_error("mnk_ls_set_option: unknown option '%s'", key);
    return -1;
}

static int ensure_wbuf(mnk_ls* ls) {
    if (ls->algo != MNK_LDL || ls->wbuf[0].p) return 0;
    const size_t cnt = (size_t)ls->ldw * std::min<int64_t>(mnk_ls_effective_nbo(ls), ls->Np) + SLACK;
    int rc = ls->wbuf[0].alloc(cnt);
    if (!rc && mnk_ls_effective_nbo(ls) < ls->Np) rc = ls->wbuf[1].alloc(cnt);
    return rc;
}

static unsigned long long* amax_word(mnk_ls* ls) {
    if (!(ls->bk_requested && ls->bk_fallback && ls->algo == MNK_LDL)) return nullptr;
    if (!ls->amax_dev.p && ls->amax_dev.alloc(AMAX_WORDS)) return nullptr;
    (void)hipMemsetAsync(ls->amax_dev.p, 0, AMAX_WORDS * sizeof(unsigned long long), ls->ctx->stream);
    return ls->amax_dev.p;
}

static int prepare_fill(mnk_ls* ls) {
    mnk_ctx* ctx = ls->ctx;
    hipStream_t s = ctx->stream;
    dim3 grid((unsigned)ls->Np, (unsigned)((ls->Np / 2 + 255) / 256));
    bool pre = ls->prefill && ls->Np <= mnk_ls::PREFILL_MAX_ROWS;
// ... 19 lines not shown
    MNK_HIP(hipGetLastError());
    return 0;
}

}
int mnk_ls_prefill_spare(mnk_ls* ls) {
    if (!ls->spare_pending) return 0;
    ls->spare_pending = false;
    if (ls->dag_filled) {
        ls->dag_filled = false;
        MNK_HIP(hipEventRecord(ls->ev_spare, ls->ctx->stream));
        ls->spare_zeroed = true;
        ls->spare_by_dag = true;
        return 0;
    }
    ls->spare_by_dag = false;
    mnk_ctx* ctx = ls->ctx;
    dim3 grid((unsigned)ls->Np, (unsigned)((ls->Np / 2 + 255) / 256));
    MNK_HIP(hipEventRecord(ls->ev_free, ctx->stream));
    MNK_HIP(hipStreamWaitEvent(ctx->s_fill, ls->ev_free, 0));
    hipLaunchKernelGGL(fill_lower_kernel, grid, dim3(256), 0, ctx->s_fill, ls->fact_spare.p, ls->ld, ls->N, ls->Np);
    MNK_HIP(hipGetLastError());
    MNK_HIP(hipEventRecord(ls->ev_spare, ctx->s_fill));
    ls->spare_zeroed = true;
    return 0;
}
extern "C" {

static int* set_envelope(mnk_ls* ls, const int32_t* env_dev, const std::vector<int32_t>& env_host, const int32_t* envh_dev,
                         const std::vector<int32_t>& envh_host) {
    ls->env_dev = nullptr;
    ls->envh_dev = nullptr;
    if (!ls->envelope || env_dev == nullptr || ls->algo == MNK_QR || ls->algo == MNK_LU || ls->algo == MNK_EVD) return nullptr;
    if (!ls->env_word.p) {
        if (ls->env_word.alloc(2) || hipMemsetAsync(ls->env_word.p, 0, 2 * sizeof(int), ls->ctx->stream) != hipSuccess) {
            (void)hipGetLastError();
            ls->env_word.release();
            return nullptr;
        }
    }
    if (ls->env_armed && hipMemsetAsync(ls->env_word.p, 0, sizeof(int), ls->ctx->stream) != hipSuccess) { (void)hipGetLastError(); return nullptr; }
    ls->env_armed = true;
    ls->env_dev = env_dev;
    ls->env_host.assign(env_host.begin(), env_host.begin() + std::min<size_t>(env_host.size(), (size_t)(ls->Np / 128)));
    if (ls->envelope_half && envh_dev != nullptr && envh_host.size() == 2 * env_host.size()) {
        ls->envh_dev = envh_dev;
        ls->envh_host.assign(envh_host.begin(), envh_host.begin() + 2 * ls->env_host.size());
    }
    return ls->env_word.p;
}

static int transfer_sc(mnk_ls* ls, mnk_sc* sc) {
    int rc = prepare_fill(ls);
    if (rc) return rc;
    const int64_t nnz = sc->nnz_aug;
    int* nonfinite = set_envelope(ls, sc->d_tile_env.p, sc->tile_env, sc->d_tile_envh.p, sc->tile_envh);
    hipLaunchKernelGGL(scatter_csc_kernel, dim3((unsigned)((nnz + 255) / 256)), dim3(256), 0, ls->ctx->stream,
                       ls->fact.p, ls->ld, sc->aug_row.p, sc->aug_col.p, sc->aug_nz.p, nnz, amax_word(ls),
                       ls->N < sc->n ? (int32_t)ls->N : INT32_MAX, nonfinite);
    MNK_HIP(hipGetLastError());
    return 0;
}

static int probe_leading_block(mnk_ls* ls, mnk_sc* sc, bool* rejected) {
    *rejected = false;
    if (!(ls->probe && ls->early_reject && ls->accept_only_pd && ls->algo == MNK_LDL && ls->N == sc->n && !mnk_batch_active())) return 0;
    if (ls->probe_last_rejected || ls->probe_hint_col < 0 || ls->probe_since_hint > 3) return 0;
    const int64_t m = (ls->probe_hint_col + 256) / 256 * 256;
    if (m < 512 || 2 * m > ls->N) return 0;
    if (ls->probe_ls == nullptr || ls->probe_order != m) {
        if (ls->probe_ls) { (void)mnk_ls_destroy(ls->probe_ls); ls->probe_ls = nullptr; }
        mnk_ls* child = nullptr;
        if (mnk_ls_create(ls->ctx, m, ls->algo, &child) != 0) { (void)hipGetLastError(); return 0; }
        child->probe = 0;
        child->accept_only_pd = 1;
        child->early_reject = 1;
        ls->probe_ls = child;
        ls->probe_order = m;
    }
    mnk_ls* c = ls->probe_ls;
    c->pivot_tol = ls->pivot_tol;
    c->envelope = ls->envelope;
    c->envelope_half = ls->envelope_half;
    if (c->dag_xcd_queues != ls->dag_xcd_queues || c->dag_gang != ls->dag_gang) {
        c->dag_xcd_queues = ls->dag_xcd_queues;
        c->dag_gang = ls->dag_gang;
        c->dag_tasks.release();
    }
    int rc = mnk_ls_factorize_sc_async(c, sc);
    if (!rc) rc = mnk_ls_fetch_info(c);
    if (rc) return rc;
    if (c->npos == m && c->nzero == 0 && c->nneg == 0) { ++ls->probe_misses; return 0; }
    ++ls->probe_hits;
    ++ls->early_rejects;
    ls->early_reject_col = c->factor_invalid ? c->early_reject_col : m - 1;
    ls->info = 1;
    ls->npos = c->npos;
    ls->nzero = c->nzero;
    ls->nneg = ls->N - ls->npos - ls->nzero;
    ls->factor_invalid = true;
    ls->info_valid = true;
    ls->factorized = true;
    ls->bk_active = false;
    ls->probe_last_rejected = true;
    if (2 * ls->early_reject_col < ls->N) { ls->probe_hint_col = ls->early_reject_col; ls->probe_since_hint = 0; }
    *rejected = true;
    return 0;
}

int mnk_ls_factorize_sc_async(mnk_ls* ls, mnk_sc* sc) {
    MNK_REQUIRE(ls && sc && sc->ctx, "mnk_ls_factorize_sc: NULL argument or host-only handle");
    MNK_REQUIRE(sc->n >= ls->N, "mnk_ls_factorize_sc: the solver's order exceeds the KKT system's");
    MNK_HIP(hipSetDevice(ls->ctx->device));
    { int rc_d = mnk_ls_sync_deferred(ls); if (rc_d) return rc_d; }
    int rc = ensure_wbuf(ls);
    if (rc) return rc;
    bool probe_rejected = false;
    rc = probe_leading_block(ls, sc, &probe_rejected);
    if (rc) return rc;
    if (!probe_rejected) {
        rc = transfer_sc(ls, sc);
        if (rc) return rc;
    }
    ls->src_persistent = true;
    ls->retransfer = [ls, sc, w = std::weak_ptr<int>(sc->alive)]() {
        if (w.expired()) {
            set_error("factorize!: the KKT handle of the last factorize! call was destroyed before its inertia was fetched; the "
                      "matrix cannot be transferred again for the fall-back tier");
            return -5;
        }
        return transfer_sc(ls, sc);
    };
    if (probe_rejected) return 0;
    return mnk_ls_run_factorization(ls);
}

static int transfer_dense(mnk_ls* ls, const double* Adev, int64_t lda) {
    ls->env_dev = nullptr;
    dim3 grid((unsigned)ls->Np, (unsigned)((ls->Np + 1023) / 1024));
    hipLaunchKernelGGL(copy_lower_kernel, grid, dim3(256), 0, ls->ctx->stream, ls->fact.p, ls->ld, Adev, lda,
                       ls->N, ls->Np, amax_word(ls));
    MNK_HIP(hipGetLastError());
    return 0;
}

static int factorize_dense_dev(mnk_ls* ls, const double* Adev, int64_t lda, bool src_persistent = false) {
    int rc = ensure_wbuf(ls);
    if (rc) return rc;
    rc = transfer_dense(ls, Adev, lda);
    if (rc) return rc;
    ls->src_persistent = src_persistent;
    ls->retransfer = [ls, Adev, lda]() { return transfer_dense(ls, Adev, lda); };
    return mnk_ls_run_factorization(ls);
}

}
int mnk_ls_factorize_dense_dev_async(mnk_ls* ls, const double* Adev, int64_t lda) {
    MNK_REQUIRE(ls && Adev && lda >= ls->N, "mnk_ls_factorize_dense_dev_async: bad argument");
    MNK_HIP(hipSetDevice(ls->ctx->device));
    { int rc_d = mnk_ls_sync_deferred(ls); if (rc_d) return rc_d; }
    return factorize_dense_dev(ls, Adev, lda);
}
extern "C" {

int mnk_ls_factorize_dc_async(mnk_ls* ls, mnk_dc* dc) {
    MNK_REQUIRE(ls && dc, "mnk_ls_factorize_dc: NULL argument");
// ... 254 lines not shown
}

int mnk_ls_solve_batch(int n, mnk_ls* const* ls, double* const* x, int loc) {
    MNK_REQUIRE(n >= 0 && (n == 0 || (ls && x)), "mnk_ls_solve_batch: NULL argument");
    int rc = mnk_solve_batch_begin();
    if (rc) return rc;
    for (int i = 0; i < n && !rc; ++i) rc = mnk_ls_solve(ls[i], x[i], 1, ls[i]->N, loc);
    const int rc_end = mnk_solve_batch_end();
    return rc ? rc : rc_end;
}

int mnk_ls_debug_dag_state(mnk_ls* ls, int* flags, int64_t nflags, int* chain, int64_t nchain, int* have) {
    MNK_REQUIRE(ls && have, "mnk_ls_debug_dag_state: NULL argument");
    *have = ls->dbg_flags.empty() ? 0 : 1;
    if (flags) memcpy(flags, ls->dbg_flags.data(), sizeof(int) * (size_t)std::min<int64_t>(nflags, (int64_t)ls->dbg_flags.size()));
    if (chain) memcpy(chain, ls->dbg_chain.data(), sizeof(int) * (size_t)std::min<int64_t>(nchain, (int64_t)ls->dbg_chain.size()));
    return 0;
}

int mnk_ls_debug_solve_trace(mnk_ls* ls, unsigned long long* out, int64_t n) {
    if (ls && out && ls->dag_trace.p && ls->dag_trace_on) {
        MNK_HIP(hipSetDevice(ls->ctx->device));
        MNK_HIP(mnk::stream_wait(ls->ctx->stream));
        const int64_t cnt = std::min<int64_t>(n, (int64_t)ls->dag_trace.n);
        MNK_HIP(mnk::d2h_copy(out, ls->dag_trace.p, cnt * sizeof(unsigned long long), ls->ctx->stream));
        return 0;
    }
    MNK_REQUIRE(ls && out && ls->solve_trace.p, "mnk_ls_debug_solve_trace: tracing is off (option solve_trace)");
    MNK_HIP(hipSetDevice(ls->ctx->device));
    MNK_HIP(mnk::stream_wait(ls->ctx->stream));
    const int64_t cnt = std::min<int64_t>(n, (ls->Np / 64) * 8);
    MNK_HIP(mnk::d2h_copy(out, ls->solve_trace.p, cnt * sizeof(unsigned long long), ls->ctx->stream));
    return 0;
}

int mnk_ls_get_factor(mnk_ls* ls, double* L, double* D, int loc) {
    MNK_REQUIRE(ls && L, "mnk_ls_get_factor: NULL argument");
    { int rc_d = mnk_ls_sync_deferred(ls); if (rc_d) return rc_d; }
    MNK_REQUIRE(ls->factorized, "mnk_ls_get_factor: factorize first");
    { int rc_f = ensure_complete_factor(ls, "mnk_ls_get_factor"); if (rc_f) return rc_f; }
    MNK_HIP(hipSetDevice(ls->ctx->device));
    hipStream_t s = ls->ctx->stream;
    if (loc == MNK_DEVICE) {
        MNK_HIP(hipMemcpy2DAsync(L, ls->N * sizeof(double), ls->fact.p, ls->ld * sizeof(double), ls->N * sizeof(double), ls->N,
                                 hipMemcpyDeviceToDevice, s));
        if (D) MNK_HIP(hipMemcpyAsync(D, ls->dvec.p, ls->N * sizeof(double), hipMemcpyDeviceToDevice, s));
        MNK_HIP(mnk::stream_wait(s));
    } else {
        MNK_HIP(mnk::d2h_copy_2d(L, ls->N * sizeof(double), ls->fact.p, ls->ld * sizeof(double), ls->N * sizeof(double), ls->N, s));
        if (D) MNK_HIP(mnk::d2h_copy(D, ls->dvec.p, ls->N * sizeof(double), s));
    }
    return 0;
}

int mnk_ls_get_stat(mnk_ls* ls, const char* key, double* value) {
    MNK_REQUIRE(ls && key && value, "mnk_ls_get_stat: NULL argument");
    MNK_HIP(hipSetDevice(ls->ctx->device));
    { int rc_d = mnk_ls_sync_deferred(ls); if (rc_d) return rc_d; }
    if (ls->factorized) {
        int rc = mnk_ls_fetch_info(ls);
        if (rc) return rc;
    }
    if (!strncmp(key, "pinned:", 7)) {
        *value = std::find(ls->env_keys.begin(), ls->env_keys.end(), std::string(key + 7)) != ls->env_keys.end() ? 1.0 : 0.0;
        return 0;
    }
    if (!strcmp(key, "panel_algo")) { *value = ls->algo_now; return 0; }
    if (!strcmp(key, "pp_fallbacks")) { *value = ls->pp_fallbacks; return 0; }
    if (!strcmp(key, "timeout_site")) { *value = ls->last_timeout_site; return 0; }
    if (!strcmp(key, "probe_hits")) { *value = (double)ls->probe_hits; return 0; }
    if (!strcmp(key, "probe_misses")) { *value = (double)ls->probe_misses; return 0; }
    if (!strcmp(key, "early_rejects")) { *value = (double)ls->early_rejects; return 0; }
    if (!strcmp(key, "early_reject_redone")) { *value = (double)ls->early_reject_redone; return 0; }
    if (!strcmp(key, "early_reject_col")) { *value = (double)ls->early_reject_col; return 0; }
    if (!strcmp(key, "stall_ms_total")) { *value = ls->stall_ms_total; return 0; }
    if (!strcmp(key, "stall_ms_process")) { *value = mnk_process_stall_ms(); return 0; }
    if (!strcmp(key, "growth")) { *value = ls->last_growth; return 0; }
    if (!strcmp(key, "sign_changes")) { *value = (double)ls->last_sign_changes; return 0; }
    if (!strcmp(key, "bk_count")) { *value = ls->bk_count; return 0; }
    if (!strcmp(key, "evd_sweeps")) { *value = ls->evd_sweeps; return 0; }
    if (!strcmp(key, "bk_panel_multi")) { *value = ls->bk_multi_last ? 1.0 : 0.0; return 0; }
    if (!strcmp(key, "bk_mw_fallbacks")) { *value = ls->bk_mw_fallbacks; return 0; }
    if (!strcmp(key, "dag_bulk_wgs")) { *value = ls->ctx->dag_cus > 0 ? mnk_ctx_bulk_wgs(ls->ctx, ls->ctx->dag_cus, 3) : 0; return 0; }
    if (!strcmp(key, "dag_ntasks")) { *value = ls->dag_ntasks; return 0; }
    if (!strcmp(key, "dag_ntasks1")) { *value = ls->dag_ntasks1; return 0; }
    if (!strcmp(key, "dag_js2")) { *value = ls->dag_js2; return 0; }
    if (!strcmp(key, "dag_nq")) { *value = std::max(ls->dag_nq[0], ls->dag_nq[1]); return 0; }
    if (!strcmp(key, "dag_steals")) {
        int st[2] = {0, 0};
        if (ls->dag_qheads.p != nullptr)
            for (int ph = 0; ph < 2; ++ph)
                MNK_HIP(mnk::d2h_copy(&st[ph], ls->dag_qheads.p + ph * mnk::DAG_QHEAD_WORDS + mnk::DAG_NQ * mnk::DAG_QHEAD_STRIDE, sizeof(int), ls->ctx->stream));
        *value = (double)st[0] + (double)st[1];
        return 0;
    }
    if (!strcmp(key, "env_ksteps") || !strcmp(key, "env_ksteps_skipped")) {
        int64_t total = 0, skipped = 0;
        int gate = 1;
        if (ls->env_used && ls->env_word.p) MNK_HIP(mnk::d2h_copy(&gate, ls->env_word.p + 1, sizeof(int), ls->ctx->stream));
        const std::vector<int>& h = ls->dag_host_tasks;
        const int ne = (int)ls->env_host.size();
        for (size_t t = 0; t + 3 < h.size(); t += 4) {
            const int flags = h[t] & 255, I = h[t + 1] & 0xffff, J = h[t + 2], kb = h[t + 3] & 0xffff, ke = h[t + 3] >> 16;
            if (flags & 8) continue;
            total += ke - kb;
            if (!ls->env_used || gate != 0 || I >= ne || J >= ne) continue;
            const int e = std::max(ls->env_host[I], ls->env_host[J]);
            skipped += std::min(ke, std::max(kb, e)) - kb;
        }
        *value = (double)(!strcmp(key, "env_ksteps") ? total : skipped);
        return 0;
    }
    if (!strcmp(key, "envh_ksteps") || !strcmp(key, "envh_ksteps_skipped")) {
        int gate = 1;
        if (ls->env_used && ls->env_word.p) MNK_HIP(mnk::d2h_copy(&gate, ls->env_word.p + 1, sizeof(int), ls->ctx->stream));
        const bool on = ls->env_used && gate == 0;
        int64_t cnt[2] = {0, 0};
        mnk::dag_envh_count(ls->dag_host_tasks, on ? ls->env_host.data() : nullptr, on && ls->envh_used ? ls->envh_host.data() : nullptr,
                            (int)ls->env_host.size(), cnt);
        *value = (double)(!strcmp(key, "envh_ksteps") ? cnt[0] : cnt[1]);
        return 0;
    }
    set_error("mnk_ls_get_stat: unknown key '%s'", key);
    return -1;
}

int mnk_ls_bk_info(mnk_ls* ls, int* active, int* count, int32_t* perm, double* doff) {
    MNK_REQUIRE(ls, "mnk_ls_bk_info: NULL argument");
    MNK_HIP(hipSetDevice(ls->ctx->device));
    { int rc_d = mnk_ls_sync_deferred(ls); if (rc_d) return rc_d; }
    if (ls->factorized) {
        int rc = mnk_ls_fetch_info(ls);
        if (rc) return rc;
    }
    if (active) *active = ls->bk_active ? 1 : 0;
    if (count) *count = ls->bk_count;
    if (ls->bk_active && (perm || doff)) {
        hipStream_t s = ls->ctx->stream;
        if (perm) MNK_HIP(mnk::d2h_copy(perm, ls->bk_perm.p, ls->N * sizeof(int32_t), s));
        if (doff) MNK_HIP(mnk::d2h_copy(doff, ls->bk_doff.p, ls->N * sizeof(double), s));
    }
    return 0;
}

int mnk_gemm_nt(mnk_ctx* ctx, int mode, int64_t M, int64_t N, int64_t K, const double* A, int64_t lda,
                const double* B, int64_t ldb, double* C, int64_t ldc) {
    MNK_REQUIRE(ctx && A && B && C, "mnk_gemm_nt: NULL argument");
    MNK_HIP(hipSetDevice(ctx->device));
    return launch_gemm_nt(ctx->stream, mode, M, N, K, A, lda, B, ldb, C, ldc, nullptr, nullptr, 0, nullptr);
}

}
```

madnlp.jl_amd/linear_solver.py:

```python
from __future__ import annotations

import atexit
import ctypes as C
import weakref
from dataclasses import dataclass

import numpy as np

from . import _lib as L

BUNCHKAUFMAN, LU, QR, CHOLESKY, LDL, EVD = "BUNCHKAUFMAN", "LU", "QR", "CHOLESKY", "LDL", "EVD"
_ALGO = {BUNCHKAUFMAN: L.MNK_BUNCHKAUFMAN, CHOLESKY: L.MNK_CHOLESKY, LDL: L.MNK_LDL, QR: L.MNK_QR, LU: L.MNK_LU, EVD: L.MNK_EVD}
_NO_INERTIA = (QR, LU)
_HIP_LINEAR_SOLVER_ALGOS = (BUNCHKAUFMAN, CHOLESKY, LDL, QR, EVD)


class LinearSolverException(Exception):
    """reference `src/LinearSolvers/linearsolvers.jl:133`."""


class SymbolicException(LinearSolverException):
    pass


# ... 27 lines not shown
            pass


class HipContext:

    def __init__(self, device: int = 0, stream: int | None = None):
        self._h = C.c_void_p()
        L.check(L.lib().mnk_ctx_create(device, C.c_void_p(stream) if stream else None, C.byref(self._h)),
                "mnk_ctx_create")
        self.device = device
        _LIVE_CONTEXTS.add(self)

    @property
    def handle(self):
        return self._h

    def synchronize(self):
        L.check(L.lib().mnk_ctx_synchronize(self._h), "mnk_ctx_synchronize")

    def stream(self) -> int:
        return L.lib().mnk_ctx_stream(self._h) or 0

    def close(self):
        if self._h:
            L.lib().mnk_ctx_destroy(self._h)
            self._h = C.c_void_p()

    def __del__(self):
        try:
            self.close()
        except Exception:
            pass


class factorize_batch:

    def __enter__(self):
        L.check(L.lib().mnk_factorize_batch_begin(), "mnk_factorize_batch_begin")
        return self

    def __exit__(self, et, ev, tb):
        rc = L.lib().mnk_factorize_batch_end()
        if rc and et is None:
            raise FactorizationException(L.lib().mnk_last_error_string().decode())
        return False


def release_idle_streams(device: int = 0):
    L.check(L.lib().mnk_release_idle_streams(int(device)), "mnk_release_idle_streams")


class solve_batch:

    def __enter__(self):
        L.check(L.lib().mnk_solve_batch_begin(), "mnk_solve_batch_begin")
        return self

    def __exit__(self, et, ev, tb):
        rc = L.lib().mnk_solve_batch_end()
        if rc and et is None:
            raise SolveException(L.lib().mnk_last_error_string().decode())
        return False


def _ptr(a):
    if a is None:
        return None, L.MNK_HOST
    if isinstance(a, np.ndarray):
        return C.c_void_p(a.ctypes.data), L.MNK_HOST
    return C.c_void_p(a.data_ptr()), (L.MNK_DEVICE if a.is_cuda else L.MNK_HOST)


@dataclass
class HipSolverOptions:
    lapack_algorithm: str = BUNCHKAUFMAN
    pivot_tol: float = 0.0
    outer_block: int = 0
    lookahead: bool = True
    share: int = 1
    small_tiles: int = 400
    persistent_solve: bool = True
    single_rows: int = 2560
    panel_algo: int = 5


class HipLinearSolver:

    _algorithms = _HIP_LINEAR_SOLVER_ALGOS

    def __init__(self, A, ctx: HipContext | None = None, opt: HipSolverOptions | None = None):
        self.opt = opt or HipSolverOptions()
        if self.opt.lapack_algorithm not in self._algorithms:
            hint = " (LU: HipLUSolver)" if self.opt.lapack_algorithm == LU else ""
            raise SymbolicException(
                f"algorithm {self.opt.lapack_algorithm} is not served by {type(self).__name__} "
                f"({', '.join(self._algorithms)}){hint}")
        self.A = A
        self.ctx = ctx or getattr(A, "ctx", None) or HipContext()
        self.n = _order_of(A)
        self._h = C.c_void_p()
        rc = L.lib().mnk_ls_create(self.ctx.handle, self.n, _ALGO[self.opt.lapack_algorithm], C.byref(self._h))
        if rc:
            raise SymbolicException(L.lib().mnk_last_error_string().decode())
        settings = [("pivot_tol", self.opt.pivot_tol), ("outer_block", self.opt.outer_block),
                    ("lookahead", float(self.opt.lookahead)), ("share", float(self.opt.share)),
                    ("small_tiles", float(self.opt.small_tiles)), ("persistent_solve", float(self.opt.persistent_solve)),
                    ("single_rows", float(self.opt.single_rows)), ("panel_algo", float(self.opt.panel_algo))]
        for key, val in settings:
            L.check(L.lib().mnk_ls_set_option(self._h, key.encode(), float(val)), "mnk_ls_set_option")
        self.info = 0
        _LIVE_OBJECTS.add(self)

    def introduce(self) -> str:
        return f"HIP-MI355X ({self.opt.lapack_algorithm})"

    def improve(self) -> bool:
        return False

    @staticmethod
    def input_type() -> str:
        return "dense"

    @staticmethod
    def default_options():
        return HipSolverOptions()

    @staticmethod
    def is_supported(dtype) -> bool:
        return np.dtype(dtype) == np.float64

    def is_inertia(self) -> bool:
        return self.opt.lapack_algorithm not in _NO_INERTIA

    def factorize(self):
        lib = L.lib()
        info = C.c_int(0)
        A = self.A
        if isinstance(A, DeviceCSC):
            rc = lib.mnk_ls_factorize_sc(self._h, A.owner_handle, C.byref(info))
        elif isinstance(A, DeviceDense):
            rc = lib.mnk_ls_factorize_dc(self._h, A.owner_handle, C.byref(info))
        elif isinstance(A, tuple):
            colptr, rowval, nzval = (np.ascontiguousarray(A[0], dtype=np.int32),
                                     np.ascontiguousarray(A[1], dtype=np.int32),
                                     np.ascontiguousarray(A[2], dtype=np.float64))
            rc = lib.mnk_ls_factorize_csc(self._h, colptr.ctypes.data, rowval.ctypes.data, nzval.ctypes.data, 0,
                                          C.byref(info))
        else:
            p, loc = _ptr(A)
            lda = A.shape[0] if isinstance(A, np.ndarray) else max(A.stride())
            if isinstance(A, np.ndarray) and not A.flags.f_contiguous:
                raise FactorizationException("dense matrices must be column-major (order='F')")
            rc = lib.mnk_ls_factorize_dense(self._h, p, lda, loc, C.byref(info))
        if rc:
            raise FactorizationException(lib.mnk_last_error_string().decode())
        self.info = info.value
        return self

    def factorize_async(self):
        lib = L.lib()
        A = self.A
        if isinstance(A, DeviceCSC):
            rc = lib.mnk_ls_factorize_sc_async(self._h, A.owner_handle)
        elif isinstance(A, DeviceDense):
            rc = lib.mnk_ls_factorize_dc_async(self._h, A.owner_handle)
        else:
            raise FactorizationException("factorize_async needs a device-resident matrix")
        if rc:
            raise FactorizationException(lib.mnk_last_error_string().decode())
        return self

    def inertia(self):
        if not self.is_inertia():
            raise InertiaException(f"{self.opt.lapack_algorithm} reveals no inertia")
        p, z, n = C.c_int64(), C.c_int64(), C.c_int64()
        rc = L.lib().mnk_ls_inertia(self._h, C.byref(p), C.byref(z), C.byref(n))
        if rc:
            raise InertiaException(L.lib().mnk_last_error_string().decode())
        return (p.value, z.value, n.value)

    def solve_linear_system(self, x):
        p, loc = _ptr(x)
        if isinstance(x, np.ndarray):
            if x.ndim == 2:
                if not x.flags.f_contiguous:
                    raise SolveException("matrix right-hand sides must be column-major")
                nrhs, ldx = x.shape[1], x.shape[0]
            else:
                if not x.flags.c_contiguous:
                    raise SolveException("x must be contiguous")
# ... 149 lines not shown
```

Baseline: 110.0 it/s.

## Build envelope-pruned task-DAG list and run it when envelope gate is open

After: 110.9 it/s (median of 6 runs). No clear change (+0.9%).

```diff
diff --git a/include/madnlp_hip.h b/include/madnlp_hip.h
--- a/include/madnlp_hip.h
+++ b/include/madnlp_hip.h
@@ -299,6 +299,8 @@
                                int* out, int cap);
 int mnk_debug_dag_deal(int ntile, int chunk, int band_tiles, int js2, int taper0, int fill, int ninst, int period, int nq, int gang,
                        int* tasks_out, int* order, int cap, int* off, int* first_phase);
+int mnk_debug_dag_pruned(int ntile, int chunk, int band_tiles, int js2, int taper0, int fill, const int* env, int nq, int gang,
+                         int* tasks_out, int* order, int cap, int* off, int* first_phase);
 
 int mnk_sc_debug_tile_env(mnk_sc* sc, int64_t order, int32_t* out, int cap);
 int mnk_debug_tile_env_csc(int64_t n, const int32_t* colptr, const int32_t* rowval, int index_base, int32_t* out, int cap);
diff --git a/madnlp.jl_amd/_lib.py b/madnlp.jl_amd/_lib.py
--- a/madnlp.jl_amd/_lib.py
+++ b/madnlp.jl_amd/_lib.py
@@ -234,6 +234,7 @@
     "mnk_debug_dag_tasks": (C.c_int, [C.c_int, C.c_int, C.c_int, C.c_int, C.c_int, _vp, C.c_int, _vp]),
     "mnk_debug_dag_merged_tasks": (C.c_int, [C.c_int] * 8 + [_vp, C.c_int]),
     "mnk_debug_dag_deal": (C.c_int, [C.c_int] * 10 + [_vp, _vp, C.c_int, _vp, _vp]),
+    "mnk_debug_dag_pruned": (C.c_int, [C.c_int] * 6 + [_vp, C.c_int, C.c_int, _vp, _vp, C.c_int, _vp, _vp]),
     "mnk_sc_debug_tile_env": (C.c_int, [_vp, C.c_int64, _vp, C.c_int]),
     "mnk_debug_tile_env_csc": (C.c_int, [C.c_int64, _vp, _vp, C.c_int, _vp, C.c_int]),
     "mnk_sc_debug_tile_envh": (C.c_int, [_vp, C.c_int64, _vp, C.c_int]),
diff --git a/madnlp.jl_amd/csrc/common.h b/madnlp.jl_amd/csrc/common.h
--- a/madnlp.jl_amd/csrc/common.h
+++ b/madnlp.jl_amd/csrc/common.h
@@ -197,7 +197,8 @@
                          const double* B, int64_t ldb, double* C, int64_t ldc, int* counter, int cus,
                          const int* info_flag);
 
-int dag_build_tasks(int ntile, int chunk, int band_tiles, int js2, std::vector<int>& out, int taper0, std::vector<int>* ready);
+int dag_build_tasks(int ntile, int chunk, int band_tiles, int js2, std::vector<int>& out, int taper0, std::vector<int>* ready,
+                    const int* env = nullptr);
 int dag_add_fill_tasks(int ntile, std::vector<int>& tasks, std::vector<int>& ready, int n1);
 void dag_merge_tasks(const std::vector<int>& tasks, const std::vector<int>& ready, int ninst, int period, std::vector<int>& out);
 constexpr int DAG_NQ = 8;
diff --git a/madnlp.jl_amd/csrc/dag.hip b/madnlp.jl_amd/csrc/dag.hip
--- a/madnlp.jl_amd/csrc/dag.hip
+++ b/madnlp.jl_amd/csrc/dag.hip
@@ -462,6 +462,10 @@
     const int* qoff;
     int* qheads;
     int nq;
+    const int4* ptasks;
+    int pntasks;
+    const int* pqoff;
+    int pnq;
 };
 
 __device__ __forceinline__ int dag_pop(const int* __restrict__ qoff, int* __restrict__ qheads, int nq, int* sq) {
@@ -493,16 +497,21 @@
     extern __shared__ __attribute__((aligned(16))) char smem_raw[];
     __shared__ int s_val;
     __shared__ int s_q[2];
+    const int* __restrict__ env = a.env != nullptr && __builtin_amdgcn_readfirstlane(*a.envgate) == 0 ? a.env : nullptr;
+    const int* __restrict__ envh = env != nullptr ? a.envh : nullptr;
+    const bool pruned = env != nullptr && a.ptasks != nullptr;
+    const int4* __restrict__ tasks = pruned ? a.ptasks : a.tasks;
+    const int ntasks = pruned ? a.pntasks : a.ntasks;
+    const int* __restrict__ qoff = pruned ? a.pqoff : a.qoff;
+    const int nq = pruned ? a.pnq : a.nq;
     if (threadIdx.x == 0) {
         unsigned xcc;
         asm volatile("s_getreg_b32 %0, hwreg(HW_REG_XCC_ID)" : "=s"(xcc));
-        s_q[0] = a.nq > 0 ? (int)(xcc & 15u) % a.nq : 0;
+        s_q[0] = nq > 0 ? (int)(xcc & 15u) % nq : 0;
         s_q[1] = 0;
     }
     __shared__ unsigned long long s_stat[4];
     if (threadIdx.x < 4) s_stat[threadIdx.x] = 0;
-    const int* __restrict__ env = a.env != nullptr && __builtin_amdgcn_readfirstlane(*a.envgate) == 0 ? a.env : nullptr;
-    const int* __restrict__ envh = env != nullptr ? a.envh : nullptr;
     __syncthreads();
     for (;;) {
         int tid = threadIdx.x;
@@ -510,26 +519,26 @@
         if (tid == 0)
             s_val = __hip_atomic_load(a.info, __ATOMIC_RELAXED, __HIP_MEMORY_SCOPE_AGENT) != 0
                         ? INT_MAX
-                        : (a.nq > 0 ? dag_pop(a.qoff, a.qheads, a.nq, s_q) : atomicAdd(a.qctr, 1));
+                        : (nq > 0 ? dag_pop(qoff, a.qheads, nq, s_q) : atomicAdd(a.qctr, 1));
         __syncthreads();
         const int t = s_val;
         __syncthreads();
-        if (t >= a.ntasks) {
+        if (t >= ntasks) {
             if (a.wgstat != nullptr && tid == 0) {
                 unsigned long long* w = a.wgstat + (int64_t)blockIdx.x * 8;
                 w[0] = s_stat[0]; w[1] = wall_clock64(); w[2] = s_stat[1]; w[3] = s_stat[2]; w[4] = s_stat[3];
-                w[5] = a.nq > 0 ? (unsigned long long)(1 + (s_q[0] >= 0 ? s_q[0] : -1 - s_q[0])) : 0; w[6] = (unsigned long long)s_q[1];
+                w[5] = nq > 0 ? (unsigned long long)(1 + (s_q[0] >= 0 ? s_q[0] : -1 - s_q[0])) : 0; w[6] = (unsigned long long)s_q[1];
             }
             return;
         }
         if (a.wgstat != nullptr && tid == 0) { if (s_stat[0] == 0) s_stat[0] = wall_clock64(); ++s_stat[2]; }
-        const int4 tk = a.tasks[t];
+        const int4 tk = tasks[t];
         const int flags = __builtin_amdgcn_readfirstlane(tk.x) & 255, q = __builtin_amdgcn_readfirstlane(tk.x) >> 8;
         const int I = __builtin_amdgcn_readfirstlane(tk.y), J = __builtin_amdgcn_readfirstlane(tk.z) & 0xfff;
         const int kbeg = __builtin_amdgcn_readfirstlane(tk.w) & 0xffff, kend = __builtin_amdgcn_readfirstlane(tk.w) >> 16;
         const int64_t row0 = (int64_t)128 * I, col0 = (int64_t)128 * J;
         unsigned long long* tr = a.trace != nullptr && tid == 0
-                                     ? a.trace + (int64_t)(a.nq > 0 ? (int)((unsigned)__builtin_amdgcn_readfirstlane(tk.z) >> 12) : t) * 8
+                                     ? a.trace + (int64_t)(nq > 0 ? (int)((unsigned)__builtin_amdgcn_readfirstlane(tk.z) >> 12) : t) * 8
                                      : nullptr;
         if (tr) { tr[0] = wall_clock64(); tr[6] = 0; tr[7] = 0; }
         if (flags & DAG_FILL) {
@@ -653,7 +662,7 @@
     }
 }
 
-int dag_build_tasks(int ntile, int chunk, int band_tiles, int js2, std::vector<int>& out, int taper0, std::vector<int>* ready) {
+int dag_build_tasks(int ntile, int chunk, int band_tiles, int js2, std::vector<int>& out, int taper0, std::vector<int>* ready, const int* env) {
     struct T { int ready, cls, J, I, flags, q, kbeg, kend; };
     std::vector<T> ts;
     auto add_tile = [&](int I, int J, int K, bool band) {
@@ -664,11 +673,14 @@
         const int first = 1 + (I * 5 + J * 3) % chunk;
         while (e > first) { e = std::max(first, e - chunk); cuts.push_back(e); }
         if (e > 0) cuts.push_back(0);
+        const int e0 = env != nullptr ? std::max(env[I], env[J]) : 0;
         int q = 0;
-        for (int c = (int)cuts.size() - 1; c > 0; --c, ++q) {
+        for (int c = (int)cuts.size() - 1; c > 0; --c) {
             const int kb = cuts[c], ke = cuts[c - 1];
             const bool last = band && ke == K;
+            if (env != nullptr && ke <= e0 && !last) continue;
             ts.push_back({ke, band ? 0 : 2, J, I, (band ? DAG_BANDACC : 0) | (last ? DAG_FINAL : 0) | (q == 0 ? DAG_FIRST : 0), q, kb, ke});
+            ++q;
         }
         if (!band) ts.push_back({K, 1, J, I, DAG_FINAL | (q == 0 ? DAG_FIRST : 0), q, body, K});
     };
@@ -837,13 +849,14 @@
 
 static int launch_dag_bulk(hipStream_t s, bool ldl, const DagInst& one, const DagInst* insts, const int* tasks, int ntasks, int ntile,
                            int* qctr, long spin_limit, int nwg, unsigned long long* trace, unsigned long long* wgstat,
-                           const int* qoff = nullptr, int* qheads = nullptr, int nq = 0) {
+                           const int* qoff = nullptr, int* qheads = nullptr, int nq = 0, const int* ptasks = nullptr, int pntasks = 0,
+                           const int* pqoff = nullptr, int pnq = 0) {
     if (ntasks <= 0) return 0;
     static const int fake = getenv("MNK_DAG_FAKE_SHARE") ? atoi(getenv("MNK_DAG_FAKE_SHARE")) : 0;
     if (insts == nullptr) {
         DagArgs1 a{one.F, one.ld, one.V, one.dinv, one.dblk, one.inv16, reinterpret_cast<const int4*>(tasks), ntasks, one.front, one.af,
                    one.tprog, ntile, qctr, one.info, spin_limit, trace, wgstat, one.vmax, fake, one.zfill, one.N, one.env, one.envgate, one.envh,
-                   qoff, qheads, nq};
+                   qoff, qheads, nq, reinterpret_cast<const int4*>(ptasks), pntasks, pqoff, pnq};
         return ldl ? launch_bulk1_t<true>(s, a, nwg) : launch_bulk1_t<false>(s, a, nwg);
     }
     DagArgs a{insts, reinterpret_cast<const int4*>(tasks), ntasks, ntile, qctr, spin_limit, trace, wgstat, fake};
@@ -905,6 +918,30 @@
     return mnk::DagInst{ls->fact.p, ls->ld, ls->algo == MNK_LDL ? ls->vfull.p : nullptr, ls->dinv.p, ls->dblk.p, ls->inv16.p,
                         front, af, tprog, ls->info_dev.p, mnk_ls_growth_word(ls), zfill, ls->N, env ? ls->env_dev : nullptr,
                         env ? ls->env_word.p + 1 : nullptr, env && ls->envelope_half ? ls->envh_dev : nullptr};
+}
+
+static void dag_device_list(const mnk_ls* ls, const std::vector<int>& h, const std::vector<int>& ready, int ntasks1, int ntile,
+                            std::vector<int>& dev_list, std::vector<int>& qoff, int* nq) {
+    const mnk_ctx* ctx = ls->ctx;
+    const int ntasks = (int)(h.size() / 4);
+    dev_list = h;
+    qoff.assign(32, 0);
+    nq[0] = nq[1] = 0;
+    if (!(ls->dag_xcd_queues && ntasks < (1 << 20) && ntile < 4096)) return;
+    const int part[3] = {0, ntasks1, ntasks};
+    const int chain_cus[2] = {ctx->dag_cus, ctx->dag_cus2};
+    for (int ph = 0; ph < 2; ++ph) {
+        const int t0 = part[ph], t1 = part[ph + 1];
+        if (t1 - t0 < mnk_ctx_bulk_wgs(ctx, chain_cus[ph], 3) || bulk_xcds(ctx, chain_cus[ph]) != mnk::DAG_NQ) continue;
+        std::vector<int> order, off;
+        mnk::dag_deal_tasks(h, ready, t0, t1, mnk::DAG_NQ, ls->dag_gang, order, off);
+        for (int p = 0; p < t1 - t0; ++p) {
+            for (int k = 0; k < 4; ++k) dev_list[4 * (size_t)(t0 + p) + k] = h[4 * (size_t)order[p] + k];
+            dev_list[4 * (size_t)(t0 + p) + 2] |= (order[p] - t0) << 12;
+        }
+        for (int x = 0; x <= mnk::DAG_NQ; ++x) qoff[16 * ph + x] = off[x];
+        nq[ph] = mnk::DAG_NQ;
+    }
 }
 
 int mnk_ls_dag_prepare(mnk_ls* ls) {
@@ -920,6 +957,8 @@
         ls->dag_flags.release();
         ls->dag_qoff.release();
         ls->dag_qheads.release();
+        ls->dag_ptasks.release();
+        ls->dag_pqoff.release();
         ls->vfull.release();
         return 1;
     };
@@ -933,24 +972,9 @@
         if (ls->dag_has_fill && h.empty()) ls->dag_has_fill = false;
         if (ls->dag_has_fill) ls->dag_ntasks1 = mnk::dag_add_fill_tasks(ntile, h, ls->dag_host_ready, ls->dag_ntasks1);
         ls->dag_ntasks = (int)(h.size() / 4);
-        std::vector<int> dev_list = h, qoff(32, 0);
-        ls->dag_nq[0] = ls->dag_nq[1] = 0;
-        if (ls->dag_xcd_queues && ls->dag_ntasks < (1 << 20) && ntile < 4096) {
-            const int part[3] = {0, ls->dag_ntasks1, ls->dag_ntasks};
-            const int chain_cus[2] = {ctx->dag_cus, ctx->dag_cus2};
-            for (int ph = 0; ph < 2; ++ph) {
-                const int t0 = part[ph], t1 = part[ph + 1];
-                if (t1 - t0 < mnk_ctx_bulk_wgs(ctx, chain_cus[ph], 3) || bulk_xcds(ctx, chain_cus[ph]) != mnk::DAG_NQ) continue;
-                std::vector<int> order, off;
-                mnk::dag_deal_tasks(h, ls->dag_host_ready, t0, t1, mnk::DAG_NQ, ls->dag_gang, order, off);
-                for (int p = 0; p < t1 - t0; ++p) {
-                    for (int k = 0; k < 4; ++k) dev_list[4 * (size_t)(t0 + p) + k] = h[4 * (size_t)order[p] + k];
-                    dev_list[4 * (size_t)(t0 + p) + 2] |= (order[p] - t0) << 12;
-                }
-                for (int x = 0; x <= mnk::DAG_NQ; ++x) qoff[16 * ph + x] = off[x];
-                ls->dag_nq[ph] = mnk::DAG_NQ;
-            }
-        }
+        std::vector<int> dev_list, qoff;
+        dag_device_list(ls, h, ls->dag_host_ready, ls->dag_ntasks1, ntile, dev_list, qoff, ls->dag_nq);
+        ls->dag_ptasks.release();
         if (ls->dag_tasks.alloc(h.size() + 4)) return give_up();
         if (!ls->dag_qoff.p && ls->dag_qoff.alloc(qoff.size())) return give_up();
         if (!ls->dag_qheads.p && ls->dag_qheads.alloc(2 * (size_t)mnk::DAG_QHEAD_WORDS)) return give_up();
@@ -961,6 +985,24 @@
             if (mnk::stream_wait(s) != hipSuccess) return give_up();
         }
         if (ls->dag_flags.alloc(nflags)) return give_up();
+    }
+    if (ls->dag_prune && ls->envelope && ls->env_dev != nullptr && ls->env_word.p != nullptr && (int)ls->env_host.size() >= ntile &&
+        ls->dag_ntasks > 0 && (!ls->dag_ptasks.p || ls->dag_penv != ls->env_host)) {
+        std::vector<int> hp, rp, dev_list, qoff;
+        ls->dag_pntasks1 = mnk::dag_build_tasks(ntile, ls->dag_chunk, ls->dag_band / 2, ls->dag_js2, hp, ls->dag_taper0, &rp, ls->env_host.data());
+        if (ls->dag_has_fill) ls->dag_pntasks1 = mnk::dag_add_fill_tasks(ntile, hp, rp, ls->dag_pntasks1);
+        ls->dag_pntasks = (int)(hp.size() / 4);
+        dag_device_list(ls, hp, rp, ls->dag_pntasks1, ntile, dev_list, qoff, ls->dag_pnq);
+        ls->dag_penv.clear();
+        if (ls->dag_ptasks.alloc(hp.size() + 4)) return give_up();
+        if (!ls->dag_pqoff.p && ls->dag_pqoff.alloc(qoff.size())) return give_up();
+        {
+            mnk::H2DGuard h2d;
+            if (hipMemcpyAsync(ls->dag_ptasks.p, dev_list.data(), dev_list.size() * sizeof(int), hipMemcpyHostToDevice, s) != hipSuccess) return give_up();
+            if (hipMemcpyAsync(ls->dag_pqoff.p, qoff.data(), qoff.size() * sizeof(int), hipMemcpyHostToDevice, s) != hipSuccess) return give_up();
+            if (mnk::stream_wait(s) != hipSuccess) return give_up();
+        }
+        ls->dag_penv = ls->env_host;
     }
     if (ldl && !ls->vfull.p && ls->vfull.alloc((size_t)ld * Np + SLACK)) {
         (void)hipGetLastError();
@@ -1006,8 +1048,11 @@
         trace = ls->dag_trace.p;
     }
     const int js2 = ls->dag_js2;
-    auto phase = [&](hipStream_t sp, hipStream_t su, int chain_cus, int task0, int ntask, int* counter, int js_begin, int js_end,
-                     unsigned strips) -> int {
+    const bool pruned = inst.env != nullptr && ls->dag_prune && trace == nullptr && ls->dag_ptasks.p != nullptr && ls->dag_pqoff.p != nullptr &&
+                        ls->dag_penv == ls->env_host;
+    ls->dag_pruned_used = pruned;
+    auto phase = [&](hipStream_t sp, hipStream_t su, int chain_cus, int task0, int ntask, int ptask0, int pntask, int* counter, int js_begin,
+                     int js_end, unsigned strips) -> int {
         const bool small = js_begin == 0 && js_end == nsc && js2 == 0;
         if (small) sp = s;
         MNK_HIP(hipEventRecord(ctx->ev_a, s));
@@ -1020,10 +1065,15 @@
         const int ph = (int)(counter - qctr), nq = ls->dag_nq[ph];
         MNK_REQUIRE(nq == 0 || (ntask >= mnk_ctx_bulk_wgs(ctx, chain_cus, 3) && bulk_xcds(ctx, chain_cus) == nq),
                     "task-DAG schedule: the bulk grid does not cover the XCDs the task list was dealt for");
+        const int pnq = pruned ? ls->dag_pnq[ph] : 0;
+        MNK_REQUIRE(pnq == 0 || (pntask >= mnk_ctx_bulk_wgs(ctx, chain_cus, 3) && bulk_xcds(ctx, chain_cus) == pnq),
+                    "task-DAG schedule: the bulk grid does not cover the XCDs the pruned task list was dealt for");
+        MNK_REQUIRE(!pruned || (pntask >= 0 && pntask <= ntask), "task-DAG schedule: the pruned list is not a part of the nominal one");
         rc = mnk::launch_dag_bulk(su, ldl, inst, nullptr, ls->dag_tasks.p + 4 * (size_t)task0, ntask, ntile, counter, spin_limit,
                                   std::min(ntask, mnk_ctx_bulk_wgs(ctx, chain_cus, 3)), trace ? trace + 8 * (size_t)task0 : nullptr,
                                   trace ? trace + (size_t)ls->dag_ntasks * 8 + 4096 * 8 + (task0 > 0 ? 512 * 8 : 0) : nullptr,
-                                  ls->dag_qoff.p + 16 * ph, ls->dag_qheads.p + ph * mnk::DAG_QHEAD_WORDS, nq);
+                                  ls->dag_qoff.p + 16 * ph, ls->dag_qheads.p + ph * mnk::DAG_QHEAD_WORDS, nq,
+                                  pruned ? ls->dag_ptasks.p + 4 * (size_t)ptask0 : nullptr, pntask, pruned ? ls->dag_pqoff.p + 16 * ph : nullptr, pnq);
         if (rc) return rc;
         if (js_begin == 0 && js_end > 0) {
             const int64_t safe = std::min<int64_t>(js_end, std::max<int64_t>(0, (ntile - ls->dag_band / 2 - 1) / 2)) & ~(int64_t)1;
@@ -1045,15 +1095,15 @@
         return 0;
     };
     if (js2 > 0) {
-        int rc = phase(ctx->sp_dag, ctx->su_dag, ctx->dag_cus, 0, ls->dag_ntasks1, qctr, 0, std::min(js2, nsc),
+        int rc = phase(ctx->sp_dag, ctx->su_dag, ctx->dag_cus, 0, ls->dag_ntasks1, 0, ls->dag_pntasks1, qctr, 0, std::min(js2, nsc),
                        (unsigned)std::min<int64_t>(ls->dag_band, Np / NBI));
         if (rc) return rc;
     }
     if (js2 < nsc) {
         const int64_t rows2 = Np - 256 * (int64_t)js2;
         MNK_REQUIRE(ctx->sp_dag2 != nullptr, "task-DAG schedule: the deep-band streams are missing");
-        int rc = phase(ctx->sp_dag2, ctx->su_dag2, ctx->dag_cus2, ls->dag_ntasks1, ls->dag_ntasks - ls->dag_ntasks1,
-                       qctr + 1, js2, nsc, (unsigned)(rows2 / NBI));
+        int rc = phase(ctx->sp_dag2, ctx->su_dag2, ctx->dag_cus2, ls->dag_ntasks1, ls->dag_ntasks - ls->dag_ntasks1, ls->dag_pntasks1,
+                       ls->dag_pntasks - ls->dag_pntasks1, qctr + 1, js2, nsc, (unsigned)(rows2 / NBI));
         if (rc) return rc;
     }
     return 0;
@@ -1472,6 +1522,31 @@
     return n;
 }
 
+extern "C" int mnk_debug_dag_pruned(int ntile, int chunk, int band_tiles, int js2, int taper0, int fill, const int* env, int nq, int gang,
+                                    int* tasks_out, int* order, int cap, int* off, int* first_phase) {
+    if (ntile <= 0 || chunk <= 0 || band_tiles <= 0 || taper0 <= 0 || nq > 64 || (nq > 0 && gang == 0)) return -1;
+    std::vector<int> h, ready;
+    int n1 = mnk::dag_build_tasks(ntile, chunk, band_tiles, js2, h, taper0, &ready, env);
+    if (fill) n1 = mnk::dag_add_fill_tasks(ntile, h, ready, n1);
+    const int n = (int)ready.size();
+    if (first_phase != nullptr) *first_phase = n1;
+    const int part[3] = {0, n1, n};
+    int written = 0;
+    for (int ph = 0; ph < 2 && nq > 0; ++ph) {
+        std::vector<int> ord, o;
+        mnk::dag_deal_tasks(h, ready, part[ph], part[ph + 1], nq, gang, ord, o);
+        for (int x = 0; x <= nq; ++x)
+            if (off != nullptr) off[ph * (nq + 1) + x] = part[ph] + o[x];
+        for (int v : ord) {
+            if (order != nullptr && written < cap) order[written] = v;
+            ++written;
+        }
+    }
+    if (tasks_out != nullptr)
+        for (int i = 0; i < std::min(n, cap) * 4; ++i) tasks_out[i] = h[i];
+    return n;
+}
+
 extern "C" int mnk_debug_envh_ksteps(int ntile, int chunk, int band_tiles, int js2, int taper0, const int* env, const int* envh, int64_t* count) {
     if (ntile <= 0 || chunk <= 0 || band_tiles <= 0 || taper0 <= 0 || count == nullptr) return -1;
     std::vector<int> h;
diff --git a/madnlp.jl_amd/csrc/factor.hip b/madnlp.jl_amd/csrc/factor.hip
--- a/madnlp.jl_amd/csrc/factor.hip
+++ b/madnlp.jl_amd/csrc/factor.hip
@@ -722,14 +722,26 @@
     unsigned long long pos = 0, zer = 0, neg = 0, chg = 0;
     double amx = 0.0;
     if (N > 0 && *info == -9) N = info[1] + 1 < N ? info[1] + 1 : N;
-    for (int64_t k = threadIdx.x; k < N; k += blockDim.x) {
-        const double d = dvec[k];
-        if (d > 0.0) ++pos;
-        else if (d < 0.0) ++neg;
-        else ++zer;
-        const double a = fabs(d) <= DBL_MAX ? fabs(d) : __longlong_as_double(0x7ff0000000000000LL);
-        amx = fmax(amx, a);
-        if (k + 1 < N && ((d > 0.0) != (dvec[k + 1] > 0.0))) ++chg;
+    for (int64_t k0 = threadIdx.x; k0 < N; k0 += 4 * (int64_t)blockDim.x) {
+        double dv[4], dn[4];
+#pragma unroll
+        for (int u = 0; u < 4; ++u) {
+            const int64_t k = k0 + u * (int64_t)blockDim.x;
+            dv[u] = k < N ? dvec[k] : 0.0;
+            dn[u] = k + 1 < N ? dvec[k + 1] : 0.0;
+        }
+#pragma unroll
+        for (int u = 0; u < 4; ++u) {
+            const int64_t k = k0 + u * (int64_t)blockDim.x;
+            if (k >= N) break;
+            const double d = dv[u];
+            if (d > 0.0) ++pos;
+            else if (d < 0.0) ++neg;
+            else ++zer;
+            const double a = fabs(d) <= DBL_MAX ? fabs(d) : __longlong_as_double(0x7ff0000000000000LL);
+            amx = fmax(amx, a);
+            if (k + 1 < N && ((d > 0.0) != (dn[u] > 0.0))) ++chg;
+        }
     }
     for (int off = 32; off > 0; off >>= 1) {
         pos += __shfl_xor((long long)pos, off);
@@ -1021,6 +1033,7 @@
     ls->algo_now = ls->panel_algo;
     ls->env_used = false;
     ls->envh_used = false;
+    ls->dag_pruned_used = false;
     const int64_t min_rows = mnk_batch_active() ? std::min<int64_t>(ls->dag_min_rows, 256) : ls->dag_min_rows;
     if (ls->algo_now == 5 && (ctx->dag_cus < ls->dag_band || !ls->lookahead || Np < min_rows || Np > ls->dag_max_rows)) ls->algo_now = 4;
     if (ls->algo_now == 5 && ctx->sp_dag == nullptr && mnk_ctx_ensure_dag(ctx) != 0) { (void)hipGetLastError(); ls->algo_now = 4; }
@@ -1195,6 +1208,11 @@
         MNK_HIP(hipStreamWaitEvent(s, ctx->ev_a, 0));
         MNK_HIP(hipStreamWaitEvent(s, ctx->ev_b, 0));
     }
+    const bool verdict_first = ls->verdict_first && ls->algo_now == 5 && ls->inv_done < (Np + 255) / 256;
+    if (verdict_first) {
+        int rc = mnk_ls_launch_finish_info(ls, s);
+        if (rc) return rc;
+    }
     {
         int rc = mnk_ls_invert_blocks(ls, s, ls->inv_done, (Np + 255) / 256);
         if (rc) return rc;
@@ -1202,7 +1220,7 @@
     ls->factorized = true;
     ls->info_valid = false;
     ls->bk_active = false;
-    {
+    if (!verdict_first) {
         int rc = mnk_ls_launch_finish_info(ls, s);
         if (rc) return rc;
     }
diff --git a/madnlp.jl_amd/csrc/ls.h b/madnlp.jl_amd/csrc/ls.h
--- a/madnlp.jl_amd/csrc/ls.h
+++ b/madnlp.jl_amd/csrc/ls.h
@@ -119,6 +119,12 @@
     int dag_nq[2] = {0, 0};
     mnk::DevBuf<int> dag_qoff;
     mnk::DevBuf<int> dag_qheads;
+    int dag_prune = 1;
+    mnk::DevBuf<int> dag_ptasks, dag_pqoff;
+    int dag_pntasks = 0, dag_pntasks1 = 0, dag_pnq[2] = {0, 0};
+    std::vector<int32_t> dag_penv;
+    bool dag_pruned_used = false;
+    int verdict_first = 0;
     mnk::DevBuf<int> dag_flags;
     mnk::DevBuf<double> vfull;
     mnk::DevBuf<unsigned long long> dag_trace;
diff --git a/madnlp.jl_amd/csrc/ls.hip b/madnlp.jl_amd/csrc/ls.hip
--- a/madnlp.jl_amd/csrc/ls.hip
+++ b/madnlp.jl_amd/csrc/ls.hip
@@ -706,6 +706,8 @@
         ls->dag_tasks.release();
         return 0;
     }
+    if (!strcmp(key, "dag_prune")) { ls->dag_prune = value != 0.0; return 0; }
+    if (!strcmp(key, "verdict_first")) { ls->verdict_first = value != 0.0; return 0; }
     if (!strcmp(key, "dag_trace")) { ls->dag_trace_on = value != 0.0; return 0; }
     if (!strcmp(key, "dag_max_rows")) { ls->dag_max_rows = (int64_t)value; return 0; }
     if (!strcmp(key, "dag_deep_rows")) { ls->dag_deep_rows = (int64_t)value; ls->dag_tasks.release(); return 0; }
@@ -891,6 +893,8 @@
     c->pivot_tol = ls->pivot_tol;
     c->envelope = ls->envelope;
     c->envelope_half = ls->envelope_half;
+    c->dag_prune = ls->dag_prune;
+    c->verdict_first = ls->verdict_first;
     if (c->dag_xcd_queues != ls->dag_xcd_queues || c->dag_gang != ls->dag_gang) {
         c->dag_xcd_queues = ls->dag_xcd_queues;
         c->dag_gang = ls->dag_gang;
@@ -1311,8 +1315,13 @@
     if (!strcmp(key, "bk_panel_multi")) { *value = ls->bk_multi_last ? 1.0 : 0.0; return 0; }
     if (!strcmp(key, "bk_mw_fallbacks")) { *value = ls->bk_mw_fallbacks; return 0; }
     if (!strcmp(key, "dag_bulk_wgs")) { *value = ls->ctx->dag_cus > 0 ? mnk_ctx_bulk_wgs(ls->ctx, ls->ctx->dag_cus, 3) : 0; return 0; }
-    if (!strcmp(key, "dag_ntasks")) { *value = ls->dag_ntasks; return 0; }
-    if (!strcmp(key, "dag_ntasks1")) { *value = ls->dag_ntasks1; return 0; }
+    if (!strcmp(key, "dag_ntasks") || !strcmp(key, "dag_ntasks1")) {
+        int gate = 1;
+        if (ls->dag_pruned_used && ls->env_word.p) MNK_HIP(mnk::d2h_copy(&gate, ls->env_word.p + 1, sizeof(int), ls->ctx->stream));
+        const bool ran_pruned = ls->dag_pruned_used && gate == 0;
+        *value = !strcmp(key, "dag_ntasks") ? (ran_pruned ? ls->dag_pntasks : ls->dag_ntasks) : (ran_pruned ? ls->dag_pntasks1 : ls->dag_ntasks1);
+        return 0;
+    }
     if (!strcmp(key, "dag_js2")) { *value = ls->dag_js2; return 0; }
     if (!strcmp(key, "dag_nq")) { *value = std::max(ls->dag_nq[0], ls->dag_nq[1]); return 0; }
     if (!strcmp(key, "dag_steals")) {
@@ -1321,6 +1330,15 @@
             for (int ph = 0; ph < 2; ++ph)
                 MNK_HIP(mnk::d2h_copy(&st[ph], ls->dag_qheads.p + ph * mnk::DAG_QHEAD_WORDS + mnk::DAG_NQ * mnk::DAG_QHEAD_STRIDE, sizeof(int), ls->ctx->stream));
         *value = (double)st[0] + (double)st[1];
+        return 0;
+    }
+    if (!strcmp(key, "dag_tasks") || !strcmp(key, "dag_tasks_pruned")) {
+        const std::vector<int>& h = ls->dag_host_tasks;
+        int64_t nominal = 0;
+        for (size_t t = 0; t + 3 < h.size(); t += 4) nominal += (h[t] & 8) ? 0 : 1;
+        int gate = 1;
+        if (ls->dag_pruned_used && ls->env_word.p) MNK_HIP(mnk::d2h_copy(&gate, ls->env_word.p + 1, sizeof(int), ls->ctx->stream));
+        *value = (double)(!strcmp(key, "dag_tasks") ? nominal : (ls->dag_pruned_used && gate == 0 ? ls->dag_ntasks - ls->dag_pntasks : 0));
         return 0;
     }
     if (!strcmp(key, "env_ksteps") || !strcmp(key, "env_ksteps_skipped")) {
diff --git a/madnlp.jl_amd/linear_solver.py b/madnlp.jl_amd/linear_solver.py
--- a/madnlp.jl_amd/linear_solver.py
+++ b/madnlp.jl_amd/linear_solver.py
@@ -133,6 +133,8 @@
     persistent_solve: bool = True
     single_rows: int = 2560
     panel_algo: int = 5
+    dag_prune: bool = True
+    verdict_first: bool = False
 
 
 class HipLinearSolver:
@@ -156,7 +158,8 @@
         settings = [("pivot_tol", self.opt.pivot_tol), ("outer_block", self.opt.outer_block),
                     ("lookahead", float(self.opt.lookahead)), ("share", float(self.opt.share)),
                     ("small_tiles", float(self.opt.small_tiles)), ("persistent_solve", float(self.opt.persistent_solve)),
-                    ("single_rows", float(self.opt.single_rows)), ("panel_algo", float(self.opt.panel_algo))]
+                    ("single_rows", float(self.opt.single_rows)), ("panel_algo", float(self.opt.panel_algo)),
+                    ("dag_prune", float(self.opt.dag_prune)), ("verdict_first", float(self.opt.verdict_first))]
         for key, val in settings:
             L.check(L.lib().mnk_ls_set_option(self._h, key.encode(), float(val)), "mnk_ls_set_option")
         self.info = 0
```
